# leijue222/Intra-and-Inter-Human-Relation-Network-for-MPEE

Measured on AMD Instinct MI355X. Metric: images/sec (256x192 crops) I2R-Net HRNet-W48 inference, higher is better.
Workload: dtype f32; 1 GPU; vanilla I2R-Net HRNet-W48-S 256x192, 6 encoder layers, fp32, random weights (BASELINE configs[1]: w48_pure_en6); images_per_gpu=8, persons_per_image=4, crops_per_gpu_step=32, parallelism=single GPU, programs_per_forward=3

## Files before the change

include/i2r_hip.h:

```cpp
#ifndef I2R_HIP_H
#define I2R_HIP_H

#include <stdint.h>

#ifdef __cplusplus
extern "C" {
#endif

#define I2R_ABI_VERSION 17

#define I2R_API __attribute__((visibility("default")))

#define I2R_OK 0
#define I2R_E_ARG (-1)
#define I2R_E_LAUNCH (-2)
#define I2R_E_NODEV (-3)

#define I2R_MAX_TAPS 9

typedef struct i2r_conv_desc {
    const float* in;
    const float* in2;
    const float* w;
    const float* bias;
    const float* res1;
    const float* res2;
    const float* res_post;
    float* out;
    int32_t n_img;
    int32_t in_h, in_w, in_cs;
    int32_t cin;
    int32_t conv_h, conv_w;
    int32_t out_h, out_w, out_cs;
    int32_t cout, cout_pad;
    int32_t stride;
    int32_t iy0, ix0;
    int32_t ntaps;
    int32_t dy[I2R_MAX_TAPS], dx[I2R_MAX_TAPS];
    int32_t out_step, out_off_y, out_off_x, rep;
    int32_t relu;
    int32_t tile_h, tile_w;
    int32_t ck;
    int32_t wn;
    int32_t mt;
    int32_t dtype;
    int32_t in_f16, out_f16;
    int32_t algo;
    int32_t t1_shift, t2_shift;
    const float* t1;
    const float* t2;
    float* y;
} i2r_conv_desc;

I2R_API int i2r_conv(const i2r_conv_desc* d, void* stream);

#define I2R_MAX_GROUP 4
I2R_API int i2r_conv_grouped(const i2r_conv_desc* const* descs, int32_t n, const int32_t* block_map, int32_t map_len,
                     void* stream);

I2R_API int i2r_stem_conv(const float* in_nchw, const float* w, const float* bias, float* out_nhwc, int32_t n_img,
                  int32_t cin, int32_t in_h, int32_t in_w, int32_t cout, int32_t out_cs, int32_t n_src, int32_t n_valid,
                  int32_t out_dt , void* stream);

I2R_API int i2r_pe_res_stem(const float* mask_nchw, const float* w_pre, const float* w7, const float* bias, float* out_nhwc,
                    int32_t n_img, int32_t in_h, int32_t in_w, int32_t cout, int32_t out_cs, int32_t n_src, int32_t n_valid, void* stream);

typedef struct i2r_pe_cat_vec_args {
    const float* in; const float* w; const float* bias; float* out;
    int32_t n_img, in_h, in_w, th, tw, rate, vec, out_cs, c0, c_end, n_src, n_valid;
} i2r_pe_cat_vec_args;
I2R_API int i2r_pe_cat_vec(const i2r_pe_cat_vec_args* a, void* stream);

I2R_API int i2r_maxpool3x3s2(const float* in, float* out, int32_t n_img, int32_t in_h, int32_t in_w, int32_t c,
                     int32_t in_cs, int32_t out_cs, void* stream);

I2R_API int i2r_head(const float* in, const float* w, const float* bias, float* out_nchw, int32_t n_img, int32_t h,
             int32_t w_, int32_t cin, int32_t in_cs, int32_t cout, void* stream);

I2R_API int i2r_conv_kernel_name(const i2r_conv_desc* const* descs, int32_t n, char* buf, int32_t buflen);

I2R_API int i2r_flip_merge(const float* y, const float* y_flipped, const int32_t* joint_map, float* out, int32_t n, int32_t joints,
                   int32_t h, int32_t w, void* stream);

I2R_API int i2r_decode(const float* heatmaps, const float* center, const float* scale, float* preds, float* maxvals, int32_t n,
               int32_t joints, int32_t h, int32_t w, int32_t blur_kernel, int32_t transform_back, void* stream);

typedef struct i2r_pose_nms_args {
    const float* preds; const float* maxvals; const float* scale; const float* area; const float* box_score;
    const int32_t* img_off; const float* sigmas;
    float* score; int32_t* rank; int32_t* n_keep;
    double in_vis_thre, oks_thre, oks_vis_thre;
    int32_t n_crops, n_img, joints, max_persons, soft, max_dets, use_oks_vis, reserved;
} i2r_pose_nms_args;
I2R_API int i2r_pose_nms(const i2r_pose_nms_args* a, void* stream);

I2R_API int i2r_group_nearest(const double* anchors, const int32_t* person_off, const int32_t* member_off, int32_t n_img, int32_t n_persons,
                              int32_t n_members, int32_t max_patch, int32_t* members, void* stream);

typedef struct i2r_oks_match_args {
    const float* dt_kpts; const float* dt_score; const uint8_t* dt_valid; const int32_t* dt_off;
    const double* gt_kpts; const double* gt_area; const double* gt_bbox; const int32_t* gt_flags; const int32_t* gt_off;
    const double* sigmas; const double* thr; const double* area_rng;
    int32_t* dt_rank; uint32_t* dt_match; uint32_t* dt_ignore; uint8_t* gt_ignore; double* oks; const int64_t* oks_off;
    int64_t oks_len;
    int32_t n_dt, n_gt, n_img, joints, n_thr, n_area, max_dets, max_dt_per_img, max_gt_per_img, reserved;
} i2r_oks_match_args;
I2R_API int i2r_oks_match(const i2r_oks_match_args* a, void* stream);

typedef struct i2r_oks_accumulate_args {
    const uint32_t* dt_match; const uint32_t* dt_ignore; const int32_t* dt_rank; const int32_t* order; const int32_t* dt_img;
    const int32_t* img_group; const uint8_t* gt_ignore; const int32_t* gt_off; const double* rec_thr;
    double* precision; double* recall; int32_t* npig;
    int32_t n_dt, n_gt, n_img, n_part, n_group, n_thr, n_area, n_rec;
} i2r_oks_accumulate_args;
I2R_API int i2r_oks_accumulate(const i2r_oks_accumulate_args* a, void* stream);

typedef struct i2r_joint_targets_args {
    const double* joints_hm; const float* joints_vis; const float* joints_weight;
    float* target_weight; float* target;
    double sigma;
    int32_t n_crops, joints, h, w;
} i2r_joint_targets_args;
I2R_API int i2r_joint_targets(const i2r_joint_targets_args* a, void* stream);

typedef struct i2r_val_metrics_args {
    const float* output;
    const float* target; const float* target_weight;
    const double* joints_hm; const float* joints_vis; const float* joints_weight;
    void* ws;
    double* loss; double* acc; double* avg_acc; int32_t* cnt; float* pred; double* sse; int32_t* hits; int32_t* valid; double* meter;
    double sigma;
    int32_t n_crops, joints, h, w, use_target_weight, reserved;
} i2r_val_metrics_args;
I2R_API int i2r_val_metrics(const i2r_val_metrics_args* a, void* stream);

I2R_API int i2r_crop_affine(const unsigned char* img, int32_t ih, int32_t iw, int32_t row_bytes, int32_t swap_rb, const float* inv_trans,
                    const float* mean, const float* inv_std, float* out, int32_t n, int32_t oh, int32_t ow, void* stream);

I2R_API int i2r_box_mask(const int32_t* boxes, int32_t ih, int32_t iw, float* out, int32_t n, int32_t oh, int32_t ow, void* stream);

I2R_API int i2r_crop_affine_cv2(const unsigned char* img, int32_t ih, int32_t iw, int32_t row_bytes, int32_t swap_rb, const double* inv_m,
                        const float* mean, const float* inv_std, float* out, int32_t n, int32_t oh, int32_t ow, void* stream);
I2R_API int i2r_box_mask_cv2(const int32_t* boxes, int32_t ih, int32_t iw, float* out, int32_t n, int32_t oh, int32_t ow, void* stream);

typedef struct {
    const unsigned char* img;
    int32_t ih, iw, row_bytes, reserved;
} i2r_image_ref;
typedef struct {
    double inv_m[6];
    int32_t box[4];
    int32_t image;
    int32_t reserved[3];
} i2r_crop_ref;
I2R_API int i2r_person_inputs_cv2(const i2r_image_ref* images, int32_t n_images, const i2r_crop_ref* crops, int32_t n_crops, int32_t swap_rb,
                          const float* mean, const float* inv_std, float* x_out, float* mask_out, int32_t oh, int32_t ow, void* stream);

I2R_API int i2r_layernorm(const float* in, const float* w, const float* b, float* out, int32_t npix, int32_t c, int32_t cs,
                  float eps, int32_t out_dt , void* stream);

I2R_API int i2r_window_attn(const float* qkv, const float* bias_qkv, float* out, int32_t n_img, int32_t h, int32_t w, int32_t c,
                    int32_t hs, int32_t heads, void* stream);

I2R_API int i2r_hrt_attn_block(const float* x, float* out, const float* ln_w, const float* ln_b, const void* wqkv, const float* bqkv,
                       const void* wo, const float* bo, int32_t n_img, int32_t h, int32_t w, int32_t c, int32_t cs, int32_t heads,
                       float eps, int32_t dtype, int32_t variant, void* stream);

I2R_API int i2r_hrt_mlp_block(const float* x, float* out, const float* ln_w, const float* ln_b, const void* w1, const float* b1,
                      const float* wdw, const float* bdw, const void* w2, const float* b2, int32_t n_img, int32_t h, int32_t w,
                      int32_t c, int32_t cs, int32_t hidden_pad, float eps, int32_t dtype, int32_t variant, void* stream);

I2R_API int i2r_dwconv3x3(const float* in, const float* w, const float* bias, float* out, int32_t n_img, int32_t in_h, int32_t in_w,
                  int32_t c, int32_t cs, int32_t stride, int32_t act, int32_t dt ,
                  void* stream);

I2R_API int i2r_upsample_bilinear_add(const float* low, const float* res, float* out, int32_t n_img, int32_t low_h, int32_t low_w,
                              int32_t scale, int32_t c, int32_t cs, int32_t act, void* stream);
struct i2r_up_args;
I2R_API int i2r_upsample_bilinear_add_multi(const struct i2r_up_args* a, void* stream);

I2R_API int i2r_fuse_up_add(const float* base, const float* t1, int32_t s1, const float* t2, int32_t s2, float* out, int32_t n_img,
                    int32_t h, int32_t w, int32_t cs, int32_t act, int32_t dt, void* stream);

typedef struct i2r_conv1x1_pair_args {
    const float* x; const float* w_a; const float* b_a; const float* res; float* y;
    const float* w_b; const float* b_b; float* z;
    int32_t n_pix, k_a, ca_out, cb_out, x_cs, y_cs, z_cs, relu_a, relu_b, mt;
} i2r_conv1x1_pair_args;
I2R_API int i2r_conv1x1_pair(const i2r_conv1x1_pair_args* a, void* stream);

typedef struct i2r_conv1x1_lp_args {
    const void* x; const void* w; const float* bias; const void* res1; const void* res_post; void* out;
    int32_t n_pix, cin_pad, cout_pad, x_cs, out_cs, act, dtype, in_16, out_16, mt;
    const void* res2;
} i2r_conv1x1_lp_args;
I2R_API int i2r_conv1x1_lp(const i2r_conv1x1_lp_args* a, void* stream);

typedef struct i2r_encoder_desc {
    const float* src;
    const float* pos;
    float* kbuf;
    float* vbuf;
    float* out;
    const int32_t* grp_off;
    const float* w_in;
    const float* b_in;
    const float* w_out;
    const float* b_out;
    const float* ln1_w; const float* ln1_b;
    const float* w1;
    const float* b1;
    const float* w2;
    const float* b2;
    const float* ln2_w; const float* ln2_b;
    int32_t n_tok, n_grp;
    int32_t d;
    int32_t cs;
    int32_t dff_pad;
    int32_t pos_period;
    int32_t n_qtiles32;
    float ln_eps;
    int32_t dtype;
    int32_t n_qtiles16, n_qtiles64;
    const void* w_in_lp; const void* w_out_lp; const void* w1_lp; const void* w2_lp;
    const float* next_w_in; const float* next_b_in; float* next_kbuf; float* next_vbuf;
    const float* vec_lp;
    float* split_ws; int32_t* split_cnt;
    int32_t n_qtiles192;
} i2r_encoder_desc;

I2R_API int i2r_encoder_kv(const i2r_encoder_desc* d, void* stream);
I2R_API int i2r_encoder_layer(const i2r_encoder_desc* d, void* stream);

typedef struct i2r_mh_attn_args {
    const float* qk; const float* v; float* out; const int32_t* grp_off;
    int32_t n_grp, heads, hp, k_off, qk_cs, v_cs, out_cs, n_qtiles16, n_qtiles32, n_qtiles64;
    const int32_t* key_len;
} i2r_mh_attn_args;
I2R_API int i2r_mh_attention(const i2r_mh_attn_args* a, void* stream);

typedef struct i2r_attn_weights_args {
    const float* qk; float* out; const int32_t* grp_off; const int64_t* out_off; float* ws;
    int32_t n_grp, heads, hp, k_off, qk_cs, n_tiles, ws_stride;
} i2r_attn_weights_args;
I2R_API int i2r_attn_weights(const i2r_attn_weights_args* a, void* stream);

typedef struct i2r_attn_query_args {
    const float* qk; float* out; const int32_t* grp_off; const int64_t* out_off; float* ws; const int32_t* q_tok; const int32_t* q_cnt;
    float* rows; const int32_t* grp_off_host;
    int32_t n_grp, heads, hp, k_off, qk_cs, n_tiles, ws_stride, mode, K, scale, h, w, n_col_tiles, reserved;
} i2r_attn_query_args;
I2R_API int i2r_attn_query_maps(const i2r_attn_query_args* a, void* stream);

I2R_API int i2r_rows_gather(const float* src, float* out, const int32_t* map, int32_t n_out, int32_t floats_per_crop, void* stream);
I2R_API int i2r_view_scramble(const float* o, float* out, const int32_t* person_map, int32_t n_out, int32_t n_images, int32_t max_persons, int32_t c,
                              int32_t cs, int32_t hw, void* stream);
typedef struct i2r_gather_args { const float* src; float* out; const int32_t* map; int32_t n_out, floats_per_crop; } i2r_gather_args;
typedef struct i2r_scramble_args { const float* o; float* out; const int32_t* person_map; int32_t n_out, n_images, max_persons, c, cs, hw; } i2r_scramble_args;

enum {
    I2R_OP_CONV = 1, I2R_OP_STEM = 2, I2R_OP_MAXPOOL = 3, I2R_OP_HEAD = 4,
    I2R_OP_ENC_KV = 5, I2R_OP_ENC_LAYER = 6, I2R_OP_FORK = 7, I2R_OP_JOIN = 8, I2R_OP_CONV_GROUP = 9,
    I2R_OP_LAYERNORM = 10, I2R_OP_WINATTN = 11, I2R_OP_DWCONV = 12, I2R_OP_UPSAMPLE = 13,
    I2R_OP_PE_RES_STEM = 15, I2R_OP_HRT_ATTN = 16, I2R_OP_HRT_MLP = 17,  I2R_OP_FUSE_UP = 19,
    I2R_OP_CONV1X1_PAIR = 20, I2R_OP_CONV1X1_LP = 21, I2R_OP_MH_ATTN = 22, I2R_OP_PE_CAT_VEC = 23, I2R_OP_ROWS_GATHER = 24, I2R_OP_VIEW_SCRAMBLE = 25,
    I2R_OP_RECORD = 26, I2R_OP_WAIT = 27, I2R_OP_LANE_FLAGS = 28, I2R_OP_ATTN_WEIGHTS = 29,
    I2R_OP_ATTN_QUERY = 30
};

typedef struct i2r_stem_args {
    const float* in; const float* w; const float* bias; float* out;
    int32_t n_img, cin, in_h, in_w, cout, out_cs, n_src, n_valid, out_dt;
} i2r_stem_args;

typedef struct i2r_pe_res_args {
    const float* in; const float* w_pre; const float* w7; const float* bias; float* out;
    int32_t n_img, in_h, in_w, cout, out_cs, n_src, n_valid;
} i2r_pe_res_args;

typedef struct i2r_pool_args {
    const float* in; float* out;
    int32_t n_img, in_h, in_w, c, in_cs, out_cs;
} i2r_pool_args;

typedef struct i2r_head_args {
    const float* in; const float* w; const float* bias; float* out;
    int32_t n_img, h, w_, cin, in_cs, cout;
} i2r_head_args;

typedef struct i2r_ln_args {
    const float* in; const float* w; const float* b; float* out;
    int32_t npix, c, cs; float eps; int32_t out_dt;
} i2r_ln_args;

typedef struct i2r_winattn_args {
    const float* qkv; const float* bias; float* out;
    int32_t n_img, h, w_, c, cs, heads;
} i2r_winattn_args;

typedef struct i2r_hrt_attn_args {
    const float* x; float* out; const float* ln_w; const float* ln_b; const void* wqkv; const float* bqkv; const void* wo; const float* bo;
    int32_t n_img, h, w_, c, cs, heads; float eps; int32_t dtype, variant;
} i2r_hrt_attn_args;

typedef struct i2r_hrt_mlp_args {
    const float* x; float* out; const float* ln_w; const float* ln_b; const void* w1; const float* b1; const float* wdw; const float* bdw;
    const void* w2; const float* b2;
    int32_t n_img, h, w_, c, cs, hidden_pad; float eps; int32_t dtype, variant;
} i2r_hrt_mlp_args;

typedef struct i2r_dw_args {
    const float* in; const float* w; const float* bias; float* out;
    int32_t n_img, in_h, in_w, c, cs, stride, act, dt;
} i2r_dw_args;

typedef struct i2r_up_args {
    const float* low; const float* res; float* out;
    int32_t n_img, low_h, low_w, scale, c, cs, act;
    const float* low2; const float* low3;
    int32_t scale2, scale3;
} i2r_up_args;

typedef struct i2r_fuse_up_args {
    const float* base; const float* t1; const float* t2; float* out;
    int32_t n_img, h, w, cs, s1, s2, act, dt;
} i2r_fuse_up_args;

typedef struct i2r_conv_group_args {
    const i2r_conv_desc* d[I2R_MAX_GROUP];
    const int32_t* block_map;
    int32_t n;
    int32_t map_len;
} i2r_conv_group_args;

typedef struct i2r_op {
    int32_t kind;
    int32_t lane;
    const void* args;
} i2r_op;

I2R_API int i2r_run_program(const i2r_op* ops, int32_t n_ops, void* const* streams, void* const* events);
I2R_API int i2r_run_program_timed(const i2r_op* ops, int32_t n_ops, void* const* streams, void* const* events, void* const* t0,
                                  void* const* t1);

I2R_API int i2r_abi_version(void);
I2R_API const char* i2r_last_error(void);
I2R_API int i2r_device_check(int32_t dev, int32_t* cu_count, int32_t* lds_bytes);

#ifdef __cplusplus
}
#endif
#endif
```

intra-and-inter-human-relation-network-for-mpee_amd/cabi.py:

```python
import ctypes as C
import os

import torch

_HERE = os.path.dirname(os.path.abspath(__file__))
LIB_PATH = os.path.join(_HERE, "libi2r_hip.so")

MAX_TAPS = 9
ABI_VERSION = 17
OP_CONV, OP_STEM, OP_MAXPOOL, OP_HEAD, OP_ENC_KV, OP_ENC_LAYER, OP_FORK, OP_JOIN, OP_CONV_GROUP = 1, 2, 3, 4, 5, 6, 7, 8, 9
MAX_GROUP = 4
OP_LAYERNORM, OP_WINATTN, OP_DWCONV, OP_UPSAMPLE = 10, 11, 12, 13
OP_CONV_CHAIN = 14
OP_PE_RES_STEM = 15
OP_HRT_ATTN = 16
OP_HRT_MLP = 17
OP_XSYNC = 18
OP_FUSE_UP = 19
OP_CONV1X1_PAIR = 20
OP_CONV1X1_LP = 21
OP_MH_ATTN = 22
OP_PE_CAT_VEC = 23
OP_ROWS_GATHER, OP_VIEW_SCRAMBLE = 24, 25
OP_RECORD, OP_WAIT = 26, 27
OP_LANE_FLAGS = 28
CAPTURE_OP_ATTN_WEIGHTS = 29
CAPTURE_OP_ATTN_QUERY = 30
SYNC_OPS = (OP_FORK, OP_JOIN, OP_XSYNC, OP_RECORD, OP_WAIT, OP_LANE_FLAGS)

_fp = C.c_void_p
_i32 = C.c_int32


class ConvDesc(C.Structure):
    _fields_ = [
        ("in_", _fp), ("in2", _fp), ("w", _fp), ("bias", _fp), ("res1", _fp), ("res2", _fp), ("res_post", _fp), ("out", _fp),
        ("n_img", _i32), ("in_h", _i32), ("in_w", _i32), ("in_cs", _i32), ("cin", _i32),
        ("conv_h", _i32), ("conv_w", _i32), ("out_h", _i32), ("out_w", _i32), ("out_cs", _i32),
        ("cout", _i32), ("cout_pad", _i32), ("stride", _i32), ("iy0", _i32), ("ix0", _i32), ("ntaps", _i32),
        ("dy", _i32 * MAX_TAPS), ("dx", _i32 * MAX_TAPS),
        ("out_step", _i32), ("out_off_y", _i32), ("out_off_x", _i32), ("rep", _i32), ("relu", _i32),
        ("tile_h", _i32), ("tile_w", _i32), ("ck", _i32), ("wn", _i32), ("mt", _i32), ("dtype", _i32),
        ("in_f16", _i32), ("out_f16", _i32), ("algo", _i32),
        ("t1_shift", _i32), ("t2_shift", _i32), ("t1", _fp), ("t2", _fp), ("y", _fp),
    ]


class EncoderDesc(C.Structure):
    _fields_ = [
        ("src", _fp), ("pos", _fp), ("kbuf", _fp), ("vbuf", _fp), ("out", _fp), ("grp_off", _fp),
        ("w_in", _fp), ("b_in", _fp), ("w_out", _fp), ("b_out", _fp), ("ln1_w", _fp), ("ln1_b", _fp),
        ("w1", _fp), ("b1", _fp), ("w2", _fp), ("b2", _fp), ("ln2_w", _fp), ("ln2_b", _fp),
        ("n_tok", _i32), ("n_grp", _i32), ("d", _i32), ("cs", _i32), ("dff_pad", _i32), ("pos_period", _i32),
        ("n_qtiles32", _i32), ("ln_eps", C.c_float), ("dtype", _i32), ("n_qtiles16", _i32), ("n_qtiles64", _i32),
        ("w_in_lp", _fp), ("w_out_lp", _fp), ("w1_lp", _fp), ("w2_lp", _fp),
        ("next_w_in", _fp), ("next_b_in", _fp), ("next_kbuf", _fp), ("next_vbuf", _fp), ("vec_lp", _fp),
        ("split_ws", _fp), ("split_cnt", _fp), ("n_qtiles192", _i32),
    ]


class StemArgs(C.Structure):
    _fields_ = [("in_", _fp), ("w", _fp), ("bias", _fp), ("out", _fp),
                ("n_img", _i32), ("cin", _i32), ("in_h", _i32), ("in_w", _i32), ("cout", _i32), ("out_cs", _i32), ("n_src", _i32),
                ("n_valid", _i32), ("out_dt", _i32)]


class PeResArgs(C.Structure):
    _fields_ = [("in_", _fp), ("w_pre", _fp), ("w7", _fp), ("bias", _fp), ("out", _fp),
                ("n_img", _i32), ("in_h", _i32), ("in_w", _i32), ("cout", _i32), ("out_cs", _i32), ("n_src", _i32), ("n_valid", _i32)]


class PeCatVecArgs(C.Structure):
    _fields_ = [("in_", _fp), ("w", _fp), ("bias", _fp), ("out", _fp),
                ("n_img", _i32), ("in_h", _i32), ("in_w", _i32), ("th", _i32), ("tw", _i32), ("rate", _i32), ("vec", _i32), ("out_cs", _i32),
                ("c0", _i32), ("c_end", _i32), ("n_src", _i32), ("n_valid", _i32)]


class PoolArgs(C.Structure):
    _fields_ = [("in_", _fp), ("out", _fp),
                ("n_img", _i32), ("in_h", _i32), ("in_w", _i32), ("c", _i32), ("in_cs", _i32), ("out_cs", _i32)]


class HeadArgs(C.Structure):
    _fields_ = [("in_", _fp), ("w", _fp), ("bias", _fp), ("out", _fp),
                ("n_img", _i32), ("h", _i32), ("w_", _i32), ("cin", _i32), ("in_cs", _i32), ("cout", _i32)]


class LnArgs(C.Structure):
    _fields_ = [("in_", _fp), ("w", _fp), ("b", _fp), ("out", _fp), ("npix", _i32), ("c", _i32), ("cs", _i32), ("eps", C.c_float),
                ("out_dt", _i32)]


class MhAttnArgs(C.Structure):
    _fields_ = [("qk", _fp), ("v", _fp), ("out", _fp), ("grp_off", _fp),
                ("n_grp", _i32), ("heads", _i32), ("hp", _i32), ("k_off", _i32), ("qk_cs", _i32), ("v_cs", _i32), ("out_cs", _i32),
                ("n_qtiles16", _i32), ("n_qtiles32", _i32), ("n_qtiles64", _i32), ("key_len", _fp)]


class AttnWeightsArgs(C.Structure):
    _fields_ = [("qk", _fp), ("out", _fp), ("grp_off", _fp), ("out_off", _fp), ("ws", _fp),
                ("n_grp", _i32), ("heads", _i32), ("hp", _i32), ("k_off", _i32), ("qk_cs", _i32), ("n_tiles", _i32), ("ws_stride", _i32)]


class AttnQueryArgs(C.Structure):
    _fields_ = [("qk", _fp), ("out", _fp), ("grp_off", _fp), ("out_off", _fp), ("ws", _fp), ("q_tok", _fp), ("q_cnt", _fp), ("rows", _fp),
                ("grp_off_host", _fp),
                ("n_grp", _i32), ("heads", _i32), ("hp", _i32), ("k_off", _i32), ("qk_cs", _i32), ("n_tiles", _i32), ("ws_stride", _i32),
                ("mode", _i32), ("K", _i32), ("scale", _i32), ("h", _i32), ("w", _i32), ("n_col_tiles", _i32), ("reserved", _i32)]


class GatherArgs(C.Structure):
    _fields_ = [("src", _fp), ("out", _fp), ("map", _fp), ("n_out", _i32), ("floats_per_crop", _i32)]


class ScrambleArgs(C.Structure):
    _fields_ = [("o", _fp), ("out", _fp), ("person_map", _fp), ("n_out", _i32), ("n_images", _i32), ("max_persons", _i32), ("c", _i32), ("cs", _i32),
                ("hw", _i32)]


class WinAttnArgs(C.Structure):
    _fields_ = [("qkv", _fp), ("bias", _fp), ("out", _fp),
                ("n_img", _i32), ("h", _i32), ("w_", _i32), ("c", _i32), ("cs", _i32), ("heads", _i32)]


class HrtAttnArgs(C.Structure):
    _fields_ = [("x", _fp), ("out", _fp), ("ln_w", _fp), ("ln_b", _fp), ("wqkv", _fp), ("bqkv", _fp), ("wo", _fp), ("bo", _fp),
                ("n_img", _i32), ("h", _i32), ("w_", _i32), ("c", _i32), ("cs", _i32), ("heads", _i32), ("eps", C.c_float), ("dtype", _i32),
                ("variant", _i32)]


class HrtMlpArgs(C.Structure):
    _fields_ = [("x", _fp), ("out", _fp), ("ln_w", _fp), ("ln_b", _fp), ("w1", _fp), ("b1", _fp), ("wdw", _fp), ("bdw", _fp), ("w2", _fp),
                ("b2", _fp), ("n_img", _i32), ("h", _i32), ("w_", _i32), ("c", _i32), ("cs", _i32), ("hidden_pad", _i32), ("eps", C.c_float),
                ("dtype", _i32), ("variant", _i32)]


class DwArgs(C.Structure):
    _fields_ = [("in_", _fp), ("w", _fp), ("bias", _fp), ("out", _fp),
                ("n_img", _i32), ("in_h", _i32), ("in_w", _i32), ("c", _i32), ("cs", _i32), ("stride", _i32), ("act", _i32), ("dt", _i32)]


class UpArgs(C.Structure):
    _fields_ = [("low", _fp), ("res", _fp), ("out", _fp),
                ("n_img", _i32), ("low_h", _i32), ("low_w", _i32), ("scale", _i32), ("c", _i32), ("cs", _i32), ("act", _i32),
                ("low2", _fp), ("low3", _fp), ("scale2", _i32), ("scale3", _i32)]


class FuseUpArgs(C.Structure):
    _fields_ = [("base", _fp), ("t1", _fp), ("t2", _fp), ("out", _fp),
                ("n_img", _i32), ("h", _i32), ("w", _i32), ("cs", _i32), ("s1", _i32), ("s2", _i32), ("act", _i32), ("dt", _i32)]


class Conv1x1PairArgs(C.Structure):
    _fields_ = [("x", _fp), ("w_a", _fp), ("b_a", _fp), ("res", _fp), ("y", _fp), ("w_b", _fp), ("b_b", _fp), ("z", _fp),
                ("n_pix", _i32), ("k_a", _i32), ("ca_out", _i32), ("cb_out", _i32), ("x_cs", _i32), ("y_cs", _i32), ("z_cs", _i32),
                ("relu_a", _i32), ("relu_b", _i32), ("mt", _i32)]


class Conv1x1LpArgs(C.Structure):
    _fields_ = [("x", _fp), ("w", _fp), ("bias", _fp), ("res1", _fp), ("res_post", _fp), ("out", _fp),
                ("n_pix", _i32), ("cin_pad", _i32), ("cout_pad", _i32), ("x_cs", _i32), ("out_cs", _i32), ("act", _i32), ("dtype", _i32),
                ("in_16", _i32), ("out_16", _i32), ("mt", _i32), ("res2", _fp)]


class ConvGroupArgs(C.Structure):
    _fields_ = [("d", C.POINTER(ConvDesc) * MAX_GROUP), ("block_map", _fp), ("n", _i32), ("map_len", _i32)]


class PoseNmsArgs(C.Structure):
    _fields_ = [("preds", _fp), ("maxvals", _fp), ("scale", _fp), ("area", _fp), ("box_score", _fp), ("img_off", _fp), ("sigmas", _fp),
                ("score", _fp), ("rank", _fp), ("n_keep", _fp),
                ("in_vis_thre", C.c_double), ("oks_thre", C.c_double), ("oks_vis_thre", C.c_double),
                ("n_crops", _i32), ("n_img", _i32), ("joints", _i32), ("max_persons", _i32), ("soft", _i32), ("max_dets", _i32),
                ("use_oks_vis", _i32), ("reserved", _i32)]


class OksMatchArgs(C.Structure):
    _fields_ = [("dt_kpts", _fp), ("dt_score", _fp), ("dt_valid", _fp), ("dt_off", _fp),
                ("gt_kpts", _fp), ("gt_area", _fp), ("gt_bbox", _fp), ("gt_flags", _fp), ("gt_off", _fp),
                ("sigmas", _fp), ("thr", _fp), ("area_rng", _fp),
                ("dt_rank", _fp), ("dt_match", _fp), ("dt_ignore", _fp), ("gt_ignore", _fp), ("oks", _fp), ("oks_off", _fp),
                ("oks_len", C.c_int64),
                ("n_dt", _i32), ("n_gt", _i32), ("n_img", _i32), ("joints", _i32), ("n_thr", _i32), ("n_area", _i32), ("max_dets", _i32),
                ("max_dt_per_img", _i32), ("max_gt_per_img", _i32), ("reserved", _i32)]


class OksAccumulateArgs(C.Structure):
    _fields_ = [("dt_match", _fp), ("dt_ignore", _fp), ("dt_rank", _fp), ("order", _fp), ("dt_img", _fp),
                ("img_group", _fp), ("gt_ignore", _fp), ("gt_off", _fp), ("rec_thr", _fp),
                ("precision", _fp), ("recall", _fp), ("npig", _fp),
                ("n_dt", _i32), ("n_gt", _i32), ("n_img", _i32), ("n_part", _i32), ("n_group", _i32), ("n_thr", _i32), ("n_area", _i32),
                ("n_rec", _i32)]


class JointTargetsArgs(C.Structure):
    _fields_ = [("joints_hm", _fp), ("joints_vis", _fp), ("joints_weight", _fp), ("target_weight", _fp), ("target", _fp),
                ("sigma", C.c_double), ("n_crops", _i32), ("joints", _i32), ("h", _i32), ("w", _i32)]


class ValMetricsArgs(C.Structure):
    _fields_ = [("output", _fp), ("target", _fp), ("target_weight", _fp), ("joints_hm", _fp), ("joints_vis", _fp), ("joints_weight", _fp),
                ("ws", _fp), ("loss", _fp), ("acc", _fp), ("avg_acc", _fp), ("cnt", _fp), ("pred", _fp), ("sse", _fp), ("hits", _fp),
                ("valid", _fp), ("meter", _fp), ("sigma", C.c_double),
                ("n_crops", _i32), ("joints", _i32), ("h", _i32), ("w", _i32), ("use_target_weight", _i32), ("reserved", _i32)]


class ImageRef(C.Structure):
    _fields_ = [("img", C.c_void_p), ("ih", _i32), ("iw", _i32), ("row_bytes", _i32), ("reserved", _i32)]


class CropRef(C.Structure):
    _fields_ = [("inv_m", C.c_double * 6), ("box", _i32 * 4), ("image", _i32), ("reserved", _i32 * 3)]


class Op(C.Structure):
    _fields_ = [("kind", _i32), ("lane", _i32), ("args", C.c_void_p)]


EXPORTS = ("i2r_conv", "i2r_conv_grouped", "i2r_conv_kernel_name", "i2r_stem_conv", "i2r_pe_res_stem", "i2r_maxpool3x3s2", "i2r_head", "i2r_layernorm", "i2r_window_attn", "i2r_hrt_attn_block", "i2r_hrt_mlp_block", "i2r_dwconv3x3",
           "i2r_upsample_bilinear_add", "i2r_upsample_bilinear_add_multi", "i2r_fuse_up_add", "i2r_conv1x1_pair", "i2r_conv1x1_lp", "i2r_flip_merge", "i2r_decode", "i2r_pose_nms", "i2r_group_nearest", "i2r_oks_match", "i2r_oks_accumulate", "i2r_joint_targets", "i2r_val_metrics", "i2r_crop_affine", "i2r_box_mask", "i2r_crop_affine_cv2", "i2r_box_mask_cv2", "i2r_person_inputs_cv2", "i2r_encoder_kv", "i2r_encoder_layer", "i2r_mh_attention", "i2r_attn_weights", "i2r_attn_query_maps", "i2r_pe_cat_vec", "i2r_rows_gather", "i2r_view_scramble",
           "i2r_run_program", "i2r_run_program_timed", "i2r_abi_version", "i2r_last_error", "i2r_device_check")

_LIB = None


class I2RError(RuntimeError):
    pass


def load_library(path=LIB_PATH):
    if not os.path.exists(path):
        raise I2RError(
            "HIP extension %s is missing -- build it with `python -c 'import __graft_entry__ as g; g.build()'`. "
            "There is no CPU fallback for the product path." % path)
    L = C.CDLL(path)
    L.i2r_conv.argtypes = [C.POINTER(ConvDesc), C.c_void_p]
    L.i2r_conv_grouped.argtypes = [C.POINTER(C.POINTER(ConvDesc)), _i32, _fp, _i32, C.c_void_p]
    L.i2r_conv_kernel_name.argtypes = [C.POINTER(C.POINTER(ConvDesc)), _i32, C.c_char_p, _i32]
    L.i2r_stem_conv.argtypes = [_fp, _fp, _fp, _fp, _i32, _i32, _i32, _i32, _i32, _i32, _i32, _i32, _i32, C.c_void_p]
    L.i2r_pe_res_stem.argtypes = [_fp, _fp, _fp, _fp, _fp, _i32, _i32, _i32, _i32, _i32, _i32, _i32, C.c_void_p]
    L.i2r_flip_merge.argtypes = [_fp, _fp, _fp, _fp, _i32, _i32, _i32, _i32, C.c_void_p]
    L.i2r_decode.argtypes = [_fp, _fp, _fp, _fp, _fp, _i32, _i32, _i32, _i32, _i32, _i32, C.c_void_p]
    L.i2r_pose_nms.argtypes = [C.POINTER(PoseNmsArgs), C.c_void_p]
    L.i2r_group_nearest.argtypes = [_fp, _fp, _fp, _i32, _i32, _i32, _i32, _fp, C.c_void_p]
    L.i2r_oks_match.argtypes = [C.POINTER(OksMatchArgs), C.c_void_p]
    L.i2r_oks_accumulate.argtypes = [C.POINTER(OksAccumulateArgs), C.c_void_p]
    L.i2r_joint_targets.argtypes = [C.POINTER(JointTargetsArgs), C.c_void_p]
    L.i2r_val_metrics.argtypes = [C.POINTER(ValMetricsArgs), C.c_void_p]
    L.i2r_crop_affine.argtypes = [_fp, _i32, _i32, _i32, _i32, _fp, _fp, _fp, _fp, _i32, _i32, _i32, C.c_void_p]
    L.i2r_box_mask.argtypes = [_fp, _i32, _i32, _fp, _i32, _i32, _i32, C.c_void_p]
    L.i2r_crop_affine_cv2.argtypes = [_fp, _i32, _i32, _i32, _i32, _fp, _fp, _fp, _fp, _i32, _i32, _i32, C.c_void_p]
    L.i2r_box_mask_cv2.argtypes = [_fp, _i32, _i32, _fp, _i32, _i32, _i32, C.c_void_p]
    L.i2r_person_inputs_cv2.argtypes = [_fp, _i32, _fp, _i32, _i32, C.POINTER(C.c_float), C.POINTER(C.c_float), _fp, _fp, _i32, _i32, C.c_void_p]
    L.i2r_fuse_up_add.argtypes = [_fp, _fp, _i32, _fp, _i32, _fp, _i32, _i32, _i32, _i32, _i32, _i32, C.c_void_p]
    L.i2r_conv1x1_pair.argtypes = [C.POINTER(Conv1x1PairArgs), C.c_void_p]
    L.i2r_conv1x1_lp.argtypes = [C.POINTER(Conv1x1LpArgs), C.c_void_p]
    L.i2r_maxpool3x3s2.argtypes = [_fp, _fp, _i32, _i32, _i32, _i32, _i32, _i32, C.c_void_p]
    L.i2r_head.argtypes = [_fp, _fp, _fp, _fp, _i32, _i32, _i32, _i32, _i32, _i32, C.c_void_p]
    L.i2r_layernorm.argtypes = [_fp, _fp, _fp, _fp, _i32, _i32, _i32, C.c_float, _i32, C.c_void_p]
    L.i2r_window_attn.argtypes = [_fp, _fp, _fp, _i32, _i32, _i32, _i32, _i32, _i32, C.c_void_p]
    L.i2r_hrt_attn_block.argtypes = [_fp, _fp, _fp, _fp, _fp, _fp, _fp, _fp, _i32, _i32, _i32, _i32, _i32, _i32, C.c_float, _i32, _i32, C.c_void_p]
    L.i2r_hrt_mlp_block.argtypes = [_fp] * 10 + [_i32] * 6 + [C.c_float, _i32, _i32, C.c_void_p]
    L.i2r_dwconv3x3.argtypes = [_fp, _fp, _fp, _fp, _i32, _i32, _i32, _i32, _i32, _i32, _i32, _i32, C.c_void_p]
    L.i2r_upsample_bilinear_add_multi.argtypes = [C.POINTER(UpArgs), C.c_void_p]
    L.i2r_upsample_bilinear_add.argtypes = [_fp, _fp, _fp, _i32, _i32, _i32, _i32, _i32, _i32, _i32, C.c_void_p]
    L.i2r_encoder_kv.argtypes = [C.POINTER(EncoderDesc), C.c_void_p]
    L.i2r_encoder_layer.argtypes = [C.POINTER(EncoderDesc), C.c_void_p]
    L.i2r_rows_gather.argtypes = [_fp, _fp, _fp, _i32, _i32, C.c_void_p]
    L.i2r_view_scramble.argtypes = [_fp, _fp, _fp, _i32, _i32, _i32, _i32, _i32, _i32, C.c_void_p]
    L.i2r_pe_cat_vec.argtypes = [C.POINTER(PeCatVecArgs), C.c_void_p]
    L.i2r_mh_attention.argtypes = [C.POINTER(MhAttnArgs), C.c_void_p]
    L.i2r_attn_weights.argtypes = [C.POINTER(AttnWeightsArgs), C.c_void_p]
    L.i2r_attn_query_maps.argtypes = [C.POINTER(AttnQueryArgs), C.c_void_p]
    L.i2r_run_program.argtypes = [C.POINTER(Op), _i32, C.POINTER(C.c_void_p), C.POINTER(C.c_void_p)]
    L.i2r_run_program_timed.argtypes = [C.POINTER(Op), _i32] + [C.POINTER(C.c_void_p)] * 4
    L.i2r_device_check.argtypes = [_i32, C.POINTER(_i32), C.POINTER(_i32)]
    L.i2r_last_error.restype = C.c_char_p
    for name in EXPORTS:
        if name != "i2r_last_error":
            getattr(L, name).restype = C.c_int
    return L


def lib():
    global _LIB
    if _LIB is None:
        L = load_library()
        if L.i2r_abi_version() != ABI_VERSION:
            raise I2RError("libi2r_hip.so ABI version %d != %d -- rebuild" % (L.i2r_abi_version(), ABI_VERSION))
        _LIB = L
    return _LIB


def check(rc, what=""):
    if rc != 0:
        msg = lib().i2r_last_error()
        raise I2RError("%s failed (rc=%d): %s" % (what or "i2r call", rc, msg.decode() if msg else "?"))


def require_gfx950(device_index=0):
    cu, lds = _i32(0), _i32(0)
    check(lib().i2r_device_check(device_index, C.byref(cu), C.byref(lds)), "i2r_device_check")
    return cu.value, lds.value
```

intra-and-inter-human-relation-network-for-mpee_amd/csrc/i2r_conv.h:

```cpp
#pragma once
#include "i2r_common.h"

#ifdef I2R_TUNING
#define I2R_DBG(p) ((p).dbg)
#else
#define I2R_DBG(p) 0
#endif

namespace {

struct ConvK {
    const float* in;
    const float* in2;
    const float* w;
    const float* bias;
    const float* res1;
    const float* res2;
    const float* res_post;
    float* out;
    int n_img, in_h, in_w, in_cs, cin;
    int conv_h, conv_w, out_h, out_w, out_cs, cout, cout_pad;
    int stride, iy0, ix0, ntaps;
    int tap_kh, tap_kw;
    int out_step, out_off_y, out_off_x, rep, relu;
    int tile_h, tile_w, tiles_y, tiles_x, n_cblk;
    int ph, pw, plane;
    int ck;
    int wn;
    int dtype;
    int in16, out16;
    int dbg;
    unsigned m_cblk, m_tx, m_ty, m_pw, m_tw;
    unsigned in_bytes, w_bytes, out_bytes;
    int wn_log, npass;
    int algo, w_fwlog, w_pitch, w_half, w_nfrag, w_rcp;
    int w_band;
    unsigned w_m_cblk, w_m_img, w_m_tx;
    const float* f_t1;
    const float* f_t2;
    float* f_y;
    int f_sh1, f_sh2;
    unsigned f_bytes1, f_bytes2;
};

__device__ __forceinline__ int div_m(int n, int d, unsigned m) { return d == 1 ? n : (int)__umulhi((unsigned)n, m); }

typedef unsigned u32x4 __attribute__((ext_vector_type(4)));
typedef unsigned u32x2 __attribute__((ext_vector_type(2)));
constexpr unsigned kOOB = 0x80000000u;
__device__ __forceinline__ __amdgpu_buffer_rsrc_t make_rsrc(const void* base, unsigned bytes) {
    return __builtin_amdgcn_make_buffer_rsrc(const_cast<void*>(base), 0, base ? bytes : 0, 0x00020000);
}
__device__ __forceinline__ f32x4 buf_ld16(const __amdgpu_buffer_rsrc_t& rs, unsigned voff, int soff) {
    return __builtin_bit_cast(f32x4, __builtin_amdgcn_raw_buffer_load_b128(rs, voff, soff, 0));
}
__device__ __forceinline__ void buf_st16(const __amdgpu_buffer_rsrc_t& rs, unsigned voff, int soff, f32x4 v) {
    __builtin_amdgcn_raw_buffer_store_b128(__builtin_bit_cast(u32x4, v), rs, voff, soff, 0);
    asm volatile("s_nop 1" ::"v"(v));
}

constexpr int kMaxPP = 5;

constexpr int kMaxGroups = 4;
struct ConvGroupK {
    ConvK g[kMaxGroups];
    int blk_end[kMaxGroups];
    int n;
    const int* blk_map;
};

template <int DT>
__device__ __forceinline__ f32x4 ld_act4(const float* base, size_t off, bool h16) {
    if constexpr (DT != 0) {
        if (h16) {
            const uint2 u = *reinterpret_cast<const uint2*>(reinterpret_cast<const unsigned short*>(base) + off);
            if constexpr (DT == 1)
                return (f32x4){__uint_as_float(u.x << 16), __uint_as_float(u.x & 0xFFFF0000u), __uint_as_float(u.y << 16), __uint_as_float(u.y & 0xFFFF0000u)};
            else {
                typedef _Float16 h4 __attribute__((ext_vector_type(4)));
                const h4 h = __builtin_bit_cast(h4, u);
                return (f32x4){(float)h[0], (float)h[1], (float)h[2], (float)h[3]};
            }
        }
    }
    return *reinterpret_cast<const f32x4*>(base + off);
}
template <int DT>
__device__ __forceinline__ void st_act4(float* base, size_t off, f32x4 v, bool h16) {
    if constexpr (DT != 0) {
        if (h16) {
            uint2 u;
            if constexpr (DT == 1) {
                typedef __bf16 b4 __attribute__((ext_vector_type(4)));
                const b4 b = {(__bf16)v[0], (__bf16)v[1], (__bf16)v[2], (__bf16)v[3]};
                u = __builtin_bit_cast(uint2, b);
            } else {
                typedef _Float16 h4 __attribute__((ext_vector_type(4)));
                const h4 h = {(_Float16)v[0], (_Float16)v[1], (_Float16)v[2], (_Float16)v[3]};
                u = __builtin_bit_cast(uint2, h);
            }
            *reinterpret_cast<uint2*>(reinterpret_cast<unsigned short*>(base) + off) = u;
            return;
        }
    }
    *reinterpret_cast<f32x4*>(base + off) = v;
}

template <int DT>
__device__ __forceinline__ f32x4 buf_ld_act4(const __amdgpu_buffer_rsrc_t& rs, unsigned voff, bool h16) {
    if constexpr (DT != 0) {
        if (h16) {
            const u32x2 u = __builtin_amdgcn_raw_buffer_load_b64(rs, voff, 0, 0);
            if constexpr (DT == 1)
                return (f32x4){__uint_as_float(u.x << 16), __uint_as_float(u.x & 0xFFFF0000u), __uint_as_float(u.y << 16), __uint_as_float(u.y & 0xFFFF0000u)};
            else {
                typedef _Float16 h4 __attribute__((ext_vector_type(4)));
                const h4 h = __builtin_bit_cast(h4, u);
                return (f32x4){(float)h[0], (float)h[1], (float)h[2], (float)h[3]};
            }
        }
    }
    return buf_ld16(rs, voff, 0);
}
template <int DT>
__device__ __forceinline__ void buf_st_act4(const __amdgpu_buffer_rsrc_t& rs, unsigned voff, f32x4 v, bool h16) {
    if constexpr (DT != 0) {
        if (h16) {
            u32x2 u;
            if constexpr (DT == 1) {
                typedef __bf16 b4 __attribute__((ext_vector_type(4)));
                const b4 b = {(__bf16)v[0], (__bf16)v[1], (__bf16)v[2], (__bf16)v[3]};
                u = __builtin_bit_cast(u32x2, b);
            } else {
                typedef _Float16 h4 __attribute__((ext_vector_type(4)));
                const h4 h = {(_Float16)v[0], (_Float16)v[1], (_Float16)v[2], (_Float16)v[3]};
                u = __builtin_bit_cast(u32x2, h);
            }
            __builtin_amdgcn_raw_buffer_store_b64(u, rs, voff, 0, 0);
            return;
        }
    }
    __builtin_amdgcn_raw_buffer_store_b128(__builtin_bit_cast(u32x4, v), rs, voff, 0, 0);
}

template <int MT, int NT, int DT>
__device__ __forceinline__ void conv_epilogue(const ConvK& p, f32x4 (&acc)[MT][NT], int img, int oy0, int ox0, int wm, int n_base,
                                              int li, int g, int tile_px) {
    if ((I2R_DBG(p) & 1) && acc[0][0][0] != 12345.678f) return;
    const int j4 = li & 3;
    const int pj = li >> 2, pq = li & 3;
    const int perm_src = (g * 16 + pq * 4 + pj) * 4;
    auto to_pixel_major = [&](f32x4 v) {
        v = quad_transpose(v, j4);
#pragma unroll
        for (int e = 0; e < 4; ++e) {
            const float x = v[e];
            v[e] = __int_as_float(__builtin_amdgcn_ds_bpermute(perm_src, __float_as_int(x)));
        }
        return v;
    };
    const bool h16 = DT != 0 && p.out16;
    const unsigned esz = h16 ? 2u : 4u;
    const __amdgpu_buffer_rsrc_t rs_out = make_rsrc(p.out, p.out_bytes), rs_r1 = make_rsrc(p.res1, p.out_bytes),
                                 rs_r2 = make_rsrc(p.res2, p.out_bytes), rs_rp = make_rsrc(p.res_post, p.out_bytes);
    auto finish = [&](f32x4 t, int n, bool full, unsigned voff) {
        if (p.relu == 1) {
            t[0] = fmaxf(t[0], 0.f); t[1] = fmaxf(t[1], 0.f); t[2] = fmaxf(t[2], 0.f); t[3] = fmaxf(t[3], 0.f);
        } else if (p.relu == 2) {
#pragma unroll
            for (int e = 0; e < 4; ++e) t[e] = 0.5f * t[e] * (1.f + erff(t[e] * 0.70710678118654752f));
        }
        if (p.res_post) t += buf_ld_act4<DT>(rs_rp, voff, h16);
        if (!full) {
#pragma unroll
            for (int e = 0; e < 4; ++e)
                if (n + e >= p.cout) t[e] = 0.f;
        }
        return t;
    };
    f32x4 bias[NT];
    unsigned noff[NT];
    const bool tail = n_base + NT * 16 > p.cout || n_base + NT * 16 > p.out_cs;
#pragma unroll
    for (int nt = 0; nt < NT; ++nt) {
        const int n = n_base + nt * 16 + pq * 4;
        const bool nok = n < p.cout_pad && (n + 4 <= p.cout || n + 4 <= p.out_cs);
        noff[nt] = nok ? (unsigned)n * esz : kOOB;
        bias[nt] = n < p.cout_pad ? *reinterpret_cast<const f32x4*>(p.bias + n) : (f32x4){0.f, 0.f, 0.f, 0.f};
    }
    if (p.rep == 1 && !(I2R_DBG(p) & 16)) {
        unsigned off[MT];
#pragma unroll
        for (int mt = 0; mt < MT; ++mt) {
            const int m = (wm * MT + mt) * 16 + g * 4 + pj;
            const int ty = div_m(m, p.tile_w, p.m_tw), tx = m - ty * p.tile_w;
            const int oy = oy0 + ty, ox = ox0 + tx;
            const bool pv = m < tile_px && oy < p.conv_h && ox < p.conv_w;
            off[mt] = pv ? (unsigned)(((img * p.out_h + oy * p.out_step + p.out_off_y) * p.out_w + ox * p.out_step + p.out_off_x) * p.out_cs) * esz : kOOB;
        }
        auto at = [&](int mt, int nt) { return (tail && noff[nt] == kOOB) ? kOOB : off[mt] + noff[nt]; };
        f32x4 r[MT][NT];
#pragma unroll
        for (int mt = 0; mt < MT; ++mt)
#pragma unroll
            for (int nt = 0; nt < NT; ++nt) {
                r[mt][nt] = bias[nt];
                if (p.res1) r[mt][nt] += buf_ld_act4<DT>(rs_r1, at(mt, nt), h16);
                if (p.res2) r[mt][nt] += buf_ld_act4<DT>(rs_r2, at(mt, nt), h16);
            }
#pragma unroll
        for (int mt = 0; mt < MT; ++mt)
#pragma unroll
            for (int nt = 0; nt < NT; ++nt) {
                const f32x4 v = to_pixel_major(acc[mt][nt]);
                const int n = n_base + nt * 16 + pq * 4;
                const unsigned o = at(mt, nt);
                buf_st_act4<DT>(rs_out, o, finish(v + r[mt][nt], n, !tail || n + 4 <= p.cout, o), h16);
            }
        return;
    }
#pragma unroll
    for (int mt = 0; mt < MT; ++mt) {
        const int m = (wm * MT + mt) * 16 + g * 4 + pj;
        const int ty = div_m(m, p.tile_w, p.m_tw), tx = m - ty * p.tile_w;
        const int oy = oy0 + ty, ox = ox0 + tx;
        const bool pvalid = m < tile_px && oy < p.conv_h && ox < p.conv_w;
        const int by = oy * p.out_step + p.out_off_y, bx = ox * p.out_step + p.out_off_x;
#pragma unroll
        for (int nt = 0; nt < NT; ++nt) {
            const f32x4 v = to_pixel_major(acc[mt][nt]) + bias[nt];
            const int n = n_base + nt * 16 + pq * 4;
            if (!pvalid || noff[nt] == kOOB) continue;
            for (int ry = 0; ry < p.rep; ++ry)
                for (int rx = 0; rx < p.rep; ++rx) {
                    const unsigned o = (unsigned)(((img * p.out_h + by + ry) * p.out_w + bx + rx) * p.out_cs) * esz + noff[nt];
                    f32x4 t = v;
                    if (p.res1) t += buf_ld_act4<DT>(rs_r1, o, h16);
                    if (p.res2) t += buf_ld_act4<DT>(rs_r2, o, h16);
                    buf_st_act4<DT>(rs_out, o, finish(t, n, n + 4 <= p.cout, o), h16);
                }
        }
    }
}



typedef void (*conv_fn)(const ConvGroupK);

}

void* i2r_pick_conv_bf16(int nt, int mt, int cap, int pf);
void* i2r_pick_conv_f16(int nt, int mt, int cap, int pf);
void* i2r_pick_conv_wino(int nt, int mt, int fin);
size_t i2r_conv_wino_lds(int nt, int mt, int plane);
```

intra-and-inter-human-relation-network-for-mpee_amd/csrc/i2r_conv.hip:

```cpp
#include <stdlib.h>

#include <algorithm>

#include "i2r_conv.h"

namespace {

template <int MT, int NT, int CAP, int PF>
__device__ __forceinline__ void conv_body(const ConvK& p, int bid, f32x4* lds) {
    const int tid = threadIdx.x;
    unsigned long long ts0 = 0, ts1 = 0, ts2 = 0;
    const bool stamp = (I2R_DBG(p) & 8) != 0;
    const int bid_stamp = bid;
    if (stamp) ts0 = __builtin_amdgcn_s_memtime();
    const int lane = tid & 63, wave = tid >> 6;
    const int WN = p.wn;
    const int wm = wave >> p.wn_log, wn = wave & (WN - 1);
    const int li = lane & 15, g = lane >> 4;

    int q = div_m(bid, p.n_cblk, p.m_cblk);
    const int cb = bid - q * p.n_cblk;
    bid = q;
    q = div_m(bid, p.tiles_x, p.m_tx);
    const int tile_x = bid - q * p.tiles_x;
    bid = q;
    const int img = div_m(bid, p.tiles_y, p.m_ty);
    const int tile_y = bid - img * p.tiles_y;
    const int oy0 = tile_y * p.tile_h, ox0 = tile_x * p.tile_w;
    const int py0 = oy0 * p.stride + p.iy0, px0 = ox0 * p.stride + p.ix0;
    const int phw = p.ph * p.pw;

    constexpr int NPP = PF > 0 ? 4 * PF : kMaxPP;
    const int ul = tid & 3;
    const __amdgpu_buffer_rsrc_t rs_in = make_rsrc(p.in, p.in_bytes), rs_in2 = make_rsrc(p.in2, p.in_bytes), rs_w = make_rsrc(p.w, p.w_bytes);
    unsigned goff[NPP];
#pragma unroll
    for (int j = 0; j < NPP; ++j) {
        const int pp = PF > 0 ? (tid >> 2) + j * 64 : tid + j * 256;
        goff[j] = kOOB;
        if (pp < phw) {
            const int py = div_m(pp, p.pw, p.m_pw), px = pp - py * p.pw;
            const int iy = py0 + py, ix = px0 + px;
            if (iy >= 0 && iy < p.in_h && ix >= 0 && ix < p.in_w) goff[j] = (unsigned)(((img * p.in_h + iy) * p.in_w + ix) * p.in_cs) * 4u;
        }
    }
    const int npp = (phw + 255) >> 8;

    const int tile_px = p.tile_h * p.tile_w;
    int ppix[MT];
#pragma unroll
    for (int mt = 0; mt < MT; ++mt) {
        int m = (wm * MT + mt) * 16 + li;
        if (m >= tile_px) m = 0;
        const int ty = div_m(m, p.tile_w, p.m_tw), tx = m - ty * p.tile_w;
        ppix[mt] = ty * p.stride * p.pw + tx * p.stride;
    }

    f32x4 acc[MT][NT];
#pragma unroll
    for (int mt = 0; mt < MT; ++mt)
#pragma unroll
        for (int nt = 0; nt < NT; ++nt) acc[mt][nt] = (f32x4){0.f, 0.f, 0.f, 0.f};

    const int n_base = (cb * WN + wn) * NT * 16;
    const int cin4 = p.cin >> 2;
    const unsigned wlane = (unsigned)(n_base + li + g * p.cout_pad) * 16u;

    auto run_chunk = [&](const f32x4* buf, int c0, int ckc, auto&& mid) {
        const int ncs = ckc >> 4;
        const int nit = p.ntaps * ncs;
        const int wp0 = (c0 >> 2) * p.cout_pad * 16;
        int wp = wp0;
        const int inc_cs = 4 * p.cout_pad * 16;
        const int inc_tap = (cin4 - (ncs - 1) * 4) * p.cout_pad * 16;
        int cs_n = 0, tx_n = 0, ty_n = 0;
        auto fetch = [&](f32x4(&a)[MT], f32x4(&b)[NT]) {
#pragma unroll
            for (int nt = 0; nt < NT; ++nt) b[nt] = buf_ld16(rs_w, wlane + nt * 256u, (I2R_DBG(p) & 4) ? wp0 : wp);
            const int abase = (cs_n * 4 + g) * p.plane + ty_n * p.pw + tx_n;
#pragma unroll
            for (int mt = 0; mt < MT; ++mt) a[mt] = buf[abase + ppix[mt]];
            if (++cs_n == ncs) {
                cs_n = 0;
                wp += inc_tap;
                if (++tx_n == p.tap_kw) {
                    tx_n = 0;
                    if (++ty_n == p.tap_kh) { ty_n = 0; wp = wp0; }
                }
            } else {
                wp += inc_cs;
            }
        };
        auto fma_step = [&](const f32x4(&a)[MT], const f32x4(&b)[NT]) {
#pragma unroll
            for (int s = 0; s < 4; ++s)
#pragma unroll
                for (int mt = 0; mt < MT; ++mt)
#pragma unroll
                    for (int nt = 0; nt < NT; ++nt) acc[mt][nt] = mfma16(a[mt][s], b[nt][s], acc[mt][nt]);
        };
        f32x4 a0[MT], a1[MT], b0[NT], b1[NT];
        fetch(a0, b0);
        mid();
        int it = 0;
        for (; it + 2 <= nit; it += 2) {
            fetch(a1, b1);
            fma_step(a0, b0);
            fetch(a0, b0);
            fma_step(a1, b1);
        }
        if (it < nit) fma_step(a0, b0);
    };

    if constexpr (PF > 0) {
        constexpr int UQ = CAP / 4, PJ = 4 * PF;
        f32x4 v[UQ][PJ];
        const int ckg = p.ck >> 2;
        auto stage_load = [&](int c0) {
#pragma unroll
            for (int uq = 0; uq < UQ; ++uq)
                if (uq * 4 < ckg) {
#pragma unroll
                    for (int j = 0; j < PJ; ++j)
                        v[uq][j] = (I2R_DBG(p) & 2) ? (f32x4){0.f, 0.f, 0.f, 0.f} : buf_ld16(rs_in, goff[j] + (uq * 4 + ul) * 16u, c0 * 4);
                }
            if (p.in2) {
#pragma unroll
                for (int uq = 0; uq < UQ; ++uq)
                    if (uq * 4 < ckg) {
#pragma unroll
                        for (int j = 0; j < PJ; ++j)
                            v[uq][j] += buf_ld16(rs_in2, goff[j] + (uq * 4 + ul) * 16u, c0 * 4);
                    }
            }
        };
        auto stage_store = [&](f32x4* buf) {
#pragma unroll
            for (int uq = 0; uq < UQ; ++uq)
                if (uq * 4 < ckg) {
#pragma unroll
                    for (int j = 0; j < PJ; ++j) {
                        const int pp = (tid >> 2) + j * 64;
                        if (pp < phw) buf[(uq * 4 + ul) * p.plane + pp] = v[uq][j];
                    }
                }
        };
        const int npass = p.npass;
        stage_load(0);
        stage_store(lds);
        __syncthreads();
        if (stamp) ts1 = __builtin_amdgcn_s_memtime();
        for (int pass = 0; pass < npass; ++pass) {
            f32x4* cur = lds + (pass & 1) * ckg * p.plane;
            f32x4* nxt = lds + ((pass + 1) & 1) * ckg * p.plane;
            const bool more = pass + 1 < npass;
            run_chunk(cur, pass * p.ck, p.ck, [&]() { if (more) stage_load((pass + 1) * p.ck); });
            if (more) stage_store(nxt);
            __syncthreads();
        }
    } else {
        for (int c0 = 0; c0 < p.cin; c0 += p.ck) {
            const int ckc = min(p.ck, p.cin - c0);
            const int ncg = ckc >> 2;
            if (c0 != 0) __syncthreads();
            for (int cg0 = 0; cg0 < ncg; cg0 += 4) {
                f32x4 v[4][kMaxPP];
#pragma unroll
                for (int u = 0; u < 4; ++u)
#pragma unroll
                    for (int j = 0; j < kMaxPP; ++j)
                        v[u][j] = (j < npp && !(I2R_DBG(p) & 2)) ? buf_ld16(rs_in, goff[j] + u * 16u, (c0 + cg0 * 4) * 4) : (f32x4){0.f, 0.f, 0.f, 0.f};
                if (p.in2) {
#pragma unroll
                    for (int u = 0; u < 4; ++u)
#pragma unroll
                        for (int j = 0; j < kMaxPP; ++j)
                            if (j < npp) v[u][j] += buf_ld16(rs_in2, goff[j] + u * 16u, (c0 + cg0 * 4) * 4);
                }
#pragma unroll
                for (int u = 0; u < 4; ++u)
#pragma unroll
                    for (int j = 0; j < kMaxPP; ++j) {
                        const int pp = tid + j * 256;
                        if (j < npp && pp < phw)
                            lds[(cg0 + u) * p.plane + pp] = v[u][j];
                    }
            }
            __syncthreads();
            run_chunk(lds, c0, ckc, []() {});
        }
    }

    if (stamp) {
        ts2 = __builtin_amdgcn_s_memtime();
        ConvK q = p;
        q.res2 = nullptr;
        conv_epilogue<MT, NT, 0>(q, acc, img, oy0, ox0, wm, n_base, li, g, tile_px);
        asm volatile("s_waitcnt vmcnt(0)" ::: "memory");
        const unsigned long long ts3 = __builtin_amdgcn_s_memtime();
        if (tid == 0) {
            unsigned long long* o = reinterpret_cast<unsigned long long*>(const_cast<float*>(p.res2)) + (size_t)bid_stamp * 4;
            o[0] = ts0; o[1] = ts1; o[2] = ts2; o[3] = ts3;
            if (I2R_DBG(p) & 32) {
                const unsigned hw = __builtin_amdgcn_s_getreg((4 << 0) | (0 << 6) | (31 << 11));
                const unsigned xcc = __builtin_amdgcn_s_getreg((20 << 0) | (0 << 6) | (3 << 11));
                o[1] = ((unsigned long long)xcc << 32) | hw;
            }
        }
        return;
    }
    conv_epilogue<MT, NT, 0>(p, acc, img, oy0, ox0, wm, n_base, li, g, tile_px);
}

template <int MT, int NT, int CAP, int PF>
__global__ __launch_bounds__(256) void conv_igemm_f32(const ConvGroupK grp) {
    extern __shared__ __attribute__((aligned(16))) f32x4 lds[];
    int bid = blockIdx.x, gi = 0, start = 0;
    if (grp.blk_map) {
        const int v = __builtin_amdgcn_readfirstlane(grp.blk_map[bid]);
        gi = v >> 24;
        bid = v & 0xFFFFFF;
    } else {
#pragma unroll
        for (int i = 0; i < kMaxGroups - 1; ++i)
            if (i + 1 < grp.n && bid >= grp.blk_end[i]) { gi = i + 1; start = grp.blk_end[i]; }
    }
    conv_body<MT, NT, CAP, PF>(grp.g[gi], bid - start, lds);
}

template <int NT, int CAP, int PF>
conv_fn pick_mt(int mt) {
    switch (mt) {
        case 1: return conv_igemm_f32<1, NT, CAP, PF>;
        case 2: return conv_igemm_f32<2, NT, CAP, PF>;
        case 3: return conv_igemm_f32<3, NT, CAP, PF>;
        case 4: return conv_igemm_f32<4, NT, CAP, PF>;
    }
    return nullptr;
}

template <int CAP, int PF>
conv_fn pick_nt(int nt, int mt) {
    switch (nt) {
        case 3: return pick_mt<3, CAP, PF>(mt);
        case 4: return pick_mt<4, CAP, PF>(mt);
        case 5: return pick_mt<5, CAP, PF>(mt);
    }
    return nullptr;
}

conv_fn pick_kernel(int nt, int mt, int cap, int pf) {
    if (pf == 0) return pick_nt<4, 0>(nt, mt);
    if (pf == 1 && cap == 4) return pick_nt<4, 1>(nt, mt);
    if (pf == 1 && cap == 12) return pick_nt<12, 1>(nt, mt);
    if (pf == 2 && cap == 4) return pick_nt<4, 2>(nt, mt);
    return nullptr;
}

inline int cdiv(int a, int b) { return (a + b - 1) / b; }

}

static void copy_desc(const i2r_conv_desc* d, ConvK& k) {
    k.in = d->in; k.in2 = d->in2; k.w = d->w; k.bias = d->bias; k.res1 = d->res1; k.res2 = d->res2; k.res_post = d->res_post; k.out = d->out;
    k.n_img = d->n_img; k.in_h = d->in_h; k.in_w = d->in_w; k.in_cs = d->in_cs; k.cin = d->cin;
    k.conv_h = d->conv_h; k.conv_w = d->conv_w; k.out_h = d->out_h; k.out_w = d->out_w; k.out_cs = d->out_cs;
    k.cout = d->cout; k.cout_pad = d->cout_pad; k.stride = d->stride; k.iy0 = d->iy0; k.ix0 = d->ix0;
    k.ntaps = d->ntaps;
    k.out_step = d->out_step; k.out_off_y = d->out_off_y; k.out_off_x = d->out_off_x; k.rep = d->rep; k.relu = d->relu;
    k.dtype = d->dtype;
    k.in16 = d->in_f16; k.out16 = d->out_f16;
    k.algo = d->algo; k.w_fwlog = k.w_pitch = k.w_half = k.w_nfrag = k.w_rcp = k.w_band = 0;
    k.w_m_cblk = k.w_m_img = k.w_m_tx = 0; k.in_bytes = k.w_bytes = k.out_bytes = 0;
    k.m_cblk = k.m_tx = k.m_ty = k.m_pw = k.m_tw = 0; k.wn_log = 0; k.npass = 0;
    k.dbg = 0;
    k.f_t1 = d->t1; k.f_t2 = d->t2; k.f_y = d->y; k.f_sh1 = d->t1_shift; k.f_sh2 = d->t2 ? d->t2_shift : 0; k.f_bytes1 = k.f_bytes2 = 0;
}

static int prepare_wino(const i2r_conv_desc* d, int force_mt, ConvK& k, int* nt_out, int* mt_out, int* cap_out, int* pf_out, size_t* lds_out,
                        long long* nblk_out) {
    I2R_CHECK_ARG(d->dtype == 0 && !d->in_f16 && !d->out_f16, "i2r_conv: the Winograd kernels are fp32");
    I2R_CHECK_ARG(d->stride == 1 && d->ntaps == 9 && d->iy0 == -1 && d->ix0 == -1 && d->rep == 1 && d->out_step == 1 && d->out_off_y == 0 &&
                      d->out_off_x == 0 && d->in2 == nullptr,
                  "i2r_conv: algo 1 (Winograd) needs a plain 3x3 stride-1 pad-1 convolution");
    for (int t = 0; t < 9; ++t) I2R_CHECK_ARG(d->dy[t] == t / 3 && d->dx[t] == t % 3, "i2r_conv: algo 1 needs row-major 3x3 taps");
    I2R_CHECK_ARG(d->relu == 0 || d->relu == 1, "i2r_conv: algo 1 has no GELU epilogue");
    I2R_CHECK_ARG((long long)d->n_img * d->in_h * d->in_w * d->in_cs < (1ll << 29) && (long long)d->n_img * d->out_h * d->out_w * d->out_cs < (1ll << 29) &&
                      (long long)16 * d->cin * d->cout_pad < (1ll << 29),
                  "i2r_conv: algo 1 addresses its tensors through buffer descriptors of < 2 GiB");
    I2R_CHECK_ARG(d->conv_h == d->in_h && d->conv_w == d->in_w && d->out_h == d->conv_h && d->out_w == d->conv_w, "i2r_conv: algo 1 geometry");
    if (d->t1) {
        I2R_CHECK_ARG(d->y != nullptr, "i2r_conv: a fused input (t1) needs y");
        I2R_CHECK_ARG(d->in_cs == d->cin, "i2r_conv: fused input: y is complete only when the conv reads every channel (cin=%d in_cs=%d)", d->cin, d->in_cs);
        for (int t = 0; t < (d->t2 ? 2 : 1); ++t) {
            const int sh = t ? d->t2_shift : d->t1_shift;
            I2R_CHECK_ARG((sh == 1 || sh == 2) && d->in_h % (1 << sh) == 0 && d->in_w % (1 << sh) == 0,
                          "i2r_conv: fused input: t%d_shift %d must be 1 or 2 and the %dx%d map divisible by the scale", t + 1, sh, d->in_h, d->in_w);
        }
        const void* others[] = {d->in, d->t1, d->t2, d->out, d->res1, d->res2, d->res_post};
        for (const void* o : others) I2R_CHECK_ARG((const void*)d->y != o, "i2r_conv: fused input: y aliases another tensor of the launch");
        I2R_CHECK_ARG(d->t1 != (const float*)d->out && d->t2 != (const float*)d->out, "i2r_conv: out aliases a fused-input term");
    }
    const int nfrag = d->cout_pad / 16;
    const int nt = nfrag % 3 == 0 ? 3 : (nfrag % 4 == 0 ? 4 : 0);
    I2R_CHECK_ARG(nt != 0, "i2r_conv: algo 1 needs cout_pad=%d to be a multiple of 48 or 64", d->cout_pad);
    const int mt = force_mt ? force_mt : (d->mt ? d->mt : 1);
    I2R_CHECK_ARG(mt == 1, "i2r_conv: algo 1 takes mt 1 (got %d)", mt);
    int fw = 0;
    if (d->tile_w) {
        I2R_CHECK_ARG(d->tile_w == 16 || d->tile_w == 8 || d->tile_w == 4, "i2r_conv: algo 1 fragment width %d (16, 8, 4)", d->tile_w);
        fw = d->tile_w / 2;
    } else {
        long long best = -1;
        for (int cand : {8, 4, 2}) {
            const long long n = (long long)cdiv(d->conv_w, 2 * cand) * cdiv(d->conv_h, 32 / cand);
            if (best < 0 || n < best) { best = n; fw = cand; }
        }
    }
    copy_desc(d, k);
    k.w_fwlog = fw == 8 ? 3 : (fw == 4 ? 2 : 1);
    k.tile_w = 2 * fw; k.tile_h = 32 / fw;
    k.tiles_x = cdiv(d->conv_w, k.tile_w); k.tiles_y = cdiv(d->conv_h, k.tile_h);
    k.n_cblk = nfrag / nt;
    k.ph = k.tile_h + 2; k.pw = k.tile_w + 2;
    k.w_half = fw + 1;
    k.w_pitch = fw == 8 ? 20 : (fw == 4 ? 10 : 9);
    k.plane = cdiv(k.ph * k.w_pitch, 16) * 16;
    k.w_rcp = (65536 + k.pw - 1) / k.pw;
    k.in_bytes = (unsigned)((long long)d->n_img * d->in_h * d->in_w * d->in_cs * 4);
    k.w_bytes = (unsigned)((long long)16 * d->cin * d->cout_pad * 4);
    k.out_bytes = (unsigned)((long long)d->n_img * d->out_h * d->out_w * d->out_cs * 4);
    if (d->t1) k.f_bytes1 = (unsigned)((long long)d->n_img * (d->in_h >> d->t1_shift) * (d->in_w >> d->t1_shift) * d->in_cs * 4);
    if (d->t2) k.f_bytes2 = (unsigned)((long long)d->n_img * (d->in_h >> d->t2_shift) * (d->in_w >> d->t2_shift) * d->in_cs * 4);
    auto magic = [](int d) { return d == 1 ? 0u : (unsigned)(((1ull << 32) + d - 1) / d); };
    k.w_m_cblk = magic(k.n_cblk); k.w_m_img = magic(k.tiles_y * k.tiles_x); k.w_m_tx = magic(k.tiles_x);
    k.tap_kw = k.tap_kh = 3;
    k.ck = 16; k.wn = 1;
    const long long nf = (long long)d->n_img * k.tiles_y * k.tiles_x;
    I2R_CHECK_ARG(nf > 0 && nf * k.n_cblk < (1ll << 20) && k.tiles_y * k.tiles_x < 2048 && k.n_cblk < 2048, "i2r_conv: algo 1 grid (%lld fragments)", nf);
    k.w_nfrag = (int)nf;
#ifdef I2R_TUNING
    {
        static const int dbg = getenv("I2R_CONV_DBG") ? atoi(getenv("I2R_CONV_DBG")) : 0;
        k.dbg = dbg;
    }
#endif
    *nt_out = nt; *mt_out = mt; *cap_out = 0; *pf_out = 100;
    *lds_out = i2r_conv_wino_lds(nt, mt, k.plane);
    *nblk_out = (nf + mt - 1) / mt * k.n_cblk;
    return I2R_OK;
}

static int prepare(const i2r_conv_desc* d, int force_mt, int force_cap, int force_pf, ConvK& k, int* nt_out, int* mt_out, int* cap_out,
                   int* pf_out, size_t* lds_out, long long* nblk_out) {
    I2R_CHECK_ARG(d && d->in && d->w && d->bias && d->out, "i2r_conv: null pointer");
    I2R_CHECK_ARG(d->cin > 0 && d->cin % 16 == 0 && d->cin <= d->in_cs && d->in_cs % 4 == 0,
                  "i2r_conv: cin=%d must be a multiple of 16 and <= in_cs=%d (in_cs %% 4 == 0)", d->cin, d->in_cs);
    I2R_CHECK_ARG(d->cout > 0 && d->cout_pad % 16 == 0 && d->cout <= d->cout_pad && d->cout <= d->out_cs && d->out_cs % 4 == 0,
                  "i2r_conv: cout=%d cout_pad=%d out_cs=%d", d->cout, d->cout_pad, d->out_cs);
    I2R_CHECK_ARG(d->stride == 1 || d->stride == 2, "i2r_conv: stride %d", d->stride);
    I2R_CHECK_ARG(d->dtype >= 0 && d->dtype <= 2 && (d->dtype == 0 || d->in2 == nullptr), "i2r_conv: dtype %d", d->dtype);
    I2R_CHECK_ARG((d->in_f16 == 0 || d->in_f16 == 1) && (d->out_f16 == 0 || d->out_f16 == 1) && (d->dtype != 0 || (!d->in_f16 && !d->out_f16)),
                  "i2r_conv: 16-bit activation storage (in_f16=%d out_f16=%d) needs a 16-bit operand type (dtype=%d)", d->in_f16, d->out_f16, d->dtype);
    I2R_CHECK_ARG(!d->in_f16 || d->in_cs % 8 == 0, "i2r_conv: 16-bit input needs in_cs %% 8 == 0 (in_cs=%d)", d->in_cs);
    I2R_CHECK_ARG(d->ntaps >= 1 && d->ntaps <= I2R_MAX_TAPS, "i2r_conv: ntaps %d", d->ntaps);
    I2R_CHECK_ARG(d->rep >= 1 && d->out_step >= 1, "i2r_conv: rep/out_step");
    I2R_CHECK_ARG((d->conv_h - 1) * d->out_step + d->out_off_y + d->rep <= d->out_h &&
                      (d->conv_w - 1) * d->out_step + d->out_off_x + d->rep <= d->out_w,
                  "i2r_conv: destination grid exceeds out tensor");
    I2R_CHECK_ARG(d->in2 != (const float*)d->out && d->in != (const float*)d->out, "i2r_conv: out aliases in");
    I2R_CHECK_ARG(d->algo == 0 || d->algo == 1, "i2r_conv: algo %d", d->algo);
    I2R_CHECK_ARG(d->t1 ? d->algo == 1 : (!d->t2 && !d->y), "i2r_conv: a fused input (t1, t2, y) needs algo 1 and starts with t1");
    if (d->algo == 1) return prepare_wino(d, force_mt, k, nt_out, mt_out, cap_out, pf_out, lds_out, nblk_out);

    int max_dy = 0, max_dx = 0;
    for (int t = 0; t < d->ntaps; ++t) {
        I2R_CHECK_ARG(d->dy[t] >= 0 && d->dx[t] >= 0, "i2r_conv: negative tap offset");
        if (d->dy[t] > max_dy) max_dy = d->dy[t];
        if (d->dx[t] > max_dx) max_dx = d->dx[t];
    }

    const int nfrag = d->cout_pad / 16;
    int nt = 0;
    for (int cand : {3, 4, 5})
        if (nfrag % cand == 0) { nt = cand; break; }
    I2R_CHECK_ARG(nt != 0, "i2r_conv: cout_pad=%d is not a multiple of 48, 64 or 80", d->cout_pad);
    int wn = d->wn;
    if (wn == 0) {
        const int nb = nfrag / nt;
        wn = (nb % 4 == 0) ? 4 : (nb % 2 == 0) ? 2 : 1;
        if (wn == 4 && d->cout_pad < 192) wn = 2;
    }
    I2R_CHECK_ARG((wn == 1 || wn == 2 || wn == 4) && (nfrag / nt) % wn == 0, "i2r_conv: wn=%d does not divide cout", wn);
    const int wm = 4 / wn;

    int th = d->tile_h, tw = d->tile_w, mt = force_mt ? force_mt : d->mt;
    if (th == 0 || tw == 0) {
        tw = d->conv_w <= 16 ? d->conv_w : (d->conv_w % 16 == 0 ? 16 : (d->conv_w % 12 == 0 ? 12 : 8));
        if (mt == 0) mt = 2;
        th = (wm * mt * 16) / tw;
        if (th < 1) th = 1;
        if (th > d->conv_h) th = d->conv_h;
    }
    if (mt == 0) mt = cdiv(th * tw, wm * 16);
    I2R_CHECK_ARG(mt >= 1 && mt <= 4 && th * tw <= wm * mt * 16, "i2r_conv: tile %dx%d does not fit wm=%d mt=%d", th, tw, wm, mt);

    copy_desc(d, k);
    k.tile_h = th; k.tile_w = tw;
    k.tiles_y = cdiv(d->conv_h, th); k.tiles_x = cdiv(d->conv_w, tw);
    k.n_cblk = nfrag / (nt * wn);
    k.ph = (th - 1) * d->stride + max_dy + 1;
    k.pw = (tw - 1) * d->stride + max_dx + 1;
    I2R_CHECK_ARG(k.ph * k.pw <= kMaxPP * 256, "i2r_conv: patch %dx%d too large", k.ph, k.pw);
#ifdef I2R_TUNING
    static const int plane_pad = getenv("I2R_CONV_PLANE_PAD") ? atoi(getenv("I2R_CONV_PLANE_PAD")) : 0;
#else
    constexpr int plane_pad = 0;
#endif
    k.plane = cdiv(k.ph * k.pw, 16) * 16 + plane_pad;
    k.tap_kw = max_dx + 1;
    k.tap_kh = max_dy + 1;
    for (int t = 0; t < d->ntaps; ++t)
        I2R_CHECK_ARG(d->dy[t] == t / k.tap_kw && d->dx[t] == t % k.tap_kw && d->ntaps == (max_dy + 1) * (max_dx + 1),
                      "i2r_conv: taps must form a dense row-major kh x kw grid");
    const int npp = cdiv(k.ph * k.pw, 256);
#ifdef I2R_TUNING
    static const int pf_env = getenv("I2R_CONV_PF") ? atoi(getenv("I2R_CONV_PF")) : 1;
#else
    constexpr int pf_env = 1;
#endif
    const int cin_g = d->dtype == 0 ? d->cin / 4 : (d->cin / 8 + 3) / 4 * 4;
    const int g_ch = d->dtype == 0 ? 4 : 8;
    int pf = (pf_env && d->ck == 0 && npp <= 2 && cin_g % 4 == 0) ? npp : 0;
    int cap = 4;
    if (force_pf >= 0) {
        I2R_CHECK_ARG(force_pf == 0 || (npp <= force_pf && d->ck == 0 && cin_g % 4 == 0), "i2r_conv: grouped members disagree on the staging mode");
        pf = force_pf;
    }
    int ck = d->ck;
    size_t lds_bytes;
    if (pf > 0) {
        int ckg = 4;
#ifdef I2R_TUNING
        static const int cap_env = getenv("I2R_CONV_CAP") ? atoi(getenv("I2R_CONV_CAP")) : 12;
#else
        constexpr int cap_env = 12;
#endif
        const int cap_max = std::min(cap_env, d->dtype == 0 ? 12 : 8);
        const int cap_lim = force_pf >= 0 ? force_cap : (pf == 1 ? cap_max : 4);
        for (int cand : {12, 8, 4})
            if (cand <= cap_lim && cin_g % cand == 0 && (size_t)2 * cand * k.plane * 16 <= 40 * 1024) { ckg = cand; break; }
        cap = force_pf >= 0 ? force_cap : (ckg > 4 ? cap_max : 4);
        ck = ckg * g_ch;
        lds_bytes = (size_t)2 * ckg * k.plane * 16;
    } else if (d->dtype != 0) {
        const int g8_pad = (d->cin / 8 + 3) / 4 * 4;
        int fit = (24 * 1024 / (k.plane * 16)) / 4 * 4;
        if (fit < 4) fit = 4;
        const int nchunk = cdiv(g8_pad, fit);
        const int ckg = cdiv(cdiv(g8_pad, nchunk), 4) * 4;
        ck = ckg * 8;
        lds_bytes = (size_t)ckg * k.plane * 16;
    } else {
        if (ck == 0) {
            const int budget = 20 * 1024;
            int fit = (budget / (k.plane * 16)) * 4;
            fit = fit < 16 ? 16 : fit / 16 * 16;
            const int nchunk = cdiv(d->cin, fit);
            ck = cdiv(cdiv(d->cin, nchunk), 16) * 16;
        }
        I2R_CHECK_ARG(ck % 16 == 0 && ck >= 16, "i2r_conv: ck=%d", ck);
        lds_bytes = (size_t)(ck / 4) * k.plane * 16;
    }
    k.ck = ck;
    I2R_CHECK_ARG(lds_bytes <= 160 * 1024, "i2r_conv: LDS %zu B", lds_bytes);
    k.wn = wn;
    {
        const long long esz_in = d->in_f16 ? 2 : 4, esz_out = d->out_f16 ? 2 : 4;
        const long long inb = (long long)d->n_img * d->in_h * d->in_w * d->in_cs * esz_in, outb = (long long)d->n_img * d->out_h * d->out_w * d->out_cs * esz_out;
        const long long wb = d->dtype == 0 ? (long long)d->ntaps * d->cin * d->cout_pad * 4 : (long long)d->ntaps * ((d->cin / 8 + 3) / 4 * 4) * 8 * d->cout_pad * 2;
        I2R_CHECK_ARG(inb < (1ll << 31) && outb < (1ll << 31) && wb < (1ll << 31), "i2r_conv: tensors of 2 GiB and more are not supported (in %lld, out %lld, weights %lld bytes)", inb, outb, wb);
        k.in_bytes = (unsigned)inb; k.out_bytes = (unsigned)outb; k.w_bytes = (unsigned)wb;
        auto magic = [](int d) { return d == 1 ? 0u : (unsigned)(((1ull << 32) + d - 1) / d); };
        k.m_cblk = magic(k.n_cblk); k.m_tx = magic(k.tiles_x); k.m_ty = magic(k.tiles_y); k.m_pw = magic(k.pw); k.m_tw = magic(k.tile_w);
        k.wn_log = wn == 4 ? 2 : (wn == 2 ? 1 : 0);
        k.npass = d->dtype == 0 ? d->cin / ck : ((d->cin / 8 + 3) / 4 * 4) / (ck / 8);
    }
#ifdef I2R_TUNING
    {
        static const int dbg = getenv("I2R_CONV_DBG") ? atoi(getenv("I2R_CONV_DBG")) : 0;
        k.dbg = dbg;
    }
#endif
    const long long nblk = (long long)d->n_img * k.tiles_y * k.tiles_x * k.n_cblk;
    I2R_CHECK_ARG(nblk > 0 && nblk < (1ll << 30), "i2r_conv: grid");
    I2R_CHECK_ARG(nblk * std::max(k.n_cblk, std::max(k.tiles_x, k.tiles_y)) < (1ll << 32) && (long long)kMaxPP * 256 * k.pw < (1ll << 32),
                  "i2r_conv: grid of %lld workgroups exceeds the index-decode range", nblk);
    *nt_out = nt; *mt_out = mt; *cap_out = cap; *pf_out = pf; *lds_out = lds_bytes; *nblk_out = nblk;
    return I2R_OK;
}

static int resolve(const i2r_conv_desc* const* descs, int32_t n, ConvGroupK& grp, int* nt0_, int* mt0_, int* cap0_, int* pf0_,
                   size_t* lds_, long long* total_, bool table = true) {
    I2R_CHECK_ARG(descs && n >= 1 && n <= kMaxGroups, "i2r_conv_grouped: 1..%d descriptors", kMaxGroups);
    int nt0 = 0, mt0 = 0, pf0 = -1, cap0 = 4;
    size_t lds_max = 0;
    long long total = 0;
    for (int i = 0; i < n; ++i) I2R_CHECK_ARG(descs[i] && descs[i]->algo == descs[0]->algo, "i2r_conv_grouped: members mix algorithms");
    if (n > 1 && descs[0]->algo == 0) {
        pf0 = 0;
        cap0 = 4;
        bool all_pf = true;
        for (int i = 0; i < n; ++i) {
            ConvK tmp;
            int nt, mt, cap, pf;
            size_t lds;
            long long nblk;
            int rc = prepare(descs[i], mt0, 4, -1, tmp, &nt, &mt, &cap, &pf, &lds, &nblk);
            if (rc) return rc;
            if (i == 0) mt0 = mt;
            if (pf == 0) all_pf = false;
            if (pf > pf0) pf0 = pf;
            if (cap > cap0) cap0 = cap;
        }
        if (!all_pf) pf0 = 0;
        if (pf0 != 1) cap0 = 4;
        mt0 = 0;
    }
    for (int i = 0; i < n; ++i) {
        int nt, mt, cap, pf;
        size_t lds;
        long long nblk;
        int rc = prepare(descs[i], mt0, cap0, pf0, grp.g[i], &nt, &mt, &cap, &pf, &lds, &nblk);
        if (rc) return rc;
        if (i == 0) { nt0 = nt; mt0 = mt; pf0 = pf; cap0 = cap; }
        I2R_CHECK_ARG(nt == nt0 && mt == mt0, "i2r_conv_grouped: descriptor %d has fragment blocking (%d,%d) != (%d,%d)", i, mt, nt, mt0, nt0);
        I2R_CHECK_ARG(descs[i]->dtype == descs[0]->dtype, "i2r_conv_grouped: members mix compute dtypes");
        if (lds > lds_max) lds_max = lds;
        if (descs[i]->algo == 1 && !table) {
            const long long groups = nblk / grp.g[i].n_cblk;
            grp.g[i].w_band = (int)((groups + 7) / 8);
            nblk = (long long)grp.g[i].w_band * 8 * grp.g[i].n_cblk;
        }
        total += nblk;
        grp.blk_end[i] = (int)total;
    }
    for (int i = n; i < kMaxGroups; ++i) { grp.g[i] = grp.g[0]; grp.blk_end[i] = (int)total; }
    grp.n = n;
    I2R_CHECK_ARG(total < (1ll << 31), "i2r_conv_grouped: grid");
    *nt0_ = nt0; *mt0_ = mt0; *cap0_ = cap0; *pf0_ = pf0; *lds_ = lds_max; *total_ = total;
    return I2R_OK;
}

static bool any_fused_input(const i2r_conv_desc* const* descs, int32_t n) {
    for (int i = 0; i < n; ++i)
        if (descs[i]->t1) return true;
    return false;
}

extern "C" int i2r_conv_grouped(const i2r_conv_desc* const* descs, int32_t n, const int32_t* block_map,
                                int32_t map_len, void* stream) {
    ConvGroupK grp;
    int nt0, mt0, cap0, pf0;
    size_t lds_max;
    long long total;
    int rc = resolve(descs, n, grp, &nt0, &mt0, &cap0, &pf0, &lds_max, &total, block_map != nullptr);
    if (rc) return rc;
    grp.blk_map = block_map;
    I2R_CHECK_ARG(block_map == nullptr || map_len == (int32_t)total, "i2r_conv_grouped: block_map has %d entries, grid has %lld", map_len, total);
    conv_fn fn = descs[0]->algo == 1 ? reinterpret_cast<conv_fn>(i2r_pick_conv_wino(nt0, mt0, any_fused_input(descs, n)))
                 : descs[0]->dtype == 0 ? pick_kernel(nt0, mt0, cap0, pf0)
                                      : reinterpret_cast<conv_fn>(descs[0]->dtype == 1 ? i2r_pick_conv_bf16(nt0, mt0, cap0, pf0) : i2r_pick_conv_f16(nt0, mt0, cap0, pf0));
    I2R_CHECK_ARG(fn != nullptr, "i2r_conv: no kernel for nt=%d mt=%d cap=%d pf=%d dtype=%d", nt0, mt0, cap0, pf0, descs[0]->dtype);
    if (lds_max > 64 * 1024)
        (void)hipFuncSetAttribute(reinterpret_cast<const void*>(fn), hipFuncAttributeMaxDynamicSharedMemorySize, (int)lds_max);
    const unsigned grid = (unsigned)total;
    i2r_launch(fn, dim3(grid), dim3(256), lds_max, (hipStream_t)stream, grp);
    I2R_CHECK_LAUNCH("i2r_conv");
    return I2R_OK;
}

extern "C" int i2r_conv(const i2r_conv_desc* d, void* stream) { return i2r_conv_grouped(&d, 1, nullptr, 0, stream); }

extern "C" int i2r_conv_kernel_name(const i2r_conv_desc* const* descs, int32_t n, char* buf, int32_t buflen) {
    ConvGroupK grp;
    int nt0, mt0, cap0, pf0;
    size_t lds_max;
    long long total;
    int rc = resolve(descs, n, grp, &nt0, &mt0, &cap0, &pf0, &lds_max, &total);
    if (rc) return rc;
    I2R_CHECK_ARG(buf && buflen > 0, "i2r_conv_kernel_name: buffer");
    if (descs[0]->algo == 1)
        snprintf(buf, (size_t)buflen, "conv_wino_%sf32<%d, %d>", any_fused_input(descs, n) ? "fin_" : "", mt0, nt0);
    else if (descs[0]->dtype)
        snprintf(buf, (size_t)buflen, "conv_igemm_lp<%d, %d, %d, %d>/%s", mt0, nt0, cap0, pf0, descs[0]->dtype == 1 ? "bf16" : "f16");
    else
        snprintf(buf, (size_t)buflen, "conv_igemm_f32<%d, %d, %d, %d>", mt0, nt0, cap0, pf0);
    return I2R_OK;
}
```

intra-and-inter-human-relation-network-for-mpee_amd/csrc/i2r_conv_wino.hip:

```cpp
#include "i2r_conv.h"

namespace {

constexpr int kWinoPatchMax = 108;

template <int MT, int NT, bool FIN>
__device__ __forceinline__ void conv_wino_body(const ConvGroupK& grp) {
    extern __shared__ __attribute__((aligned(16))) f32x4 lds[];
    const int tid = threadIdx.x, lane = tid & 63;
    const int wi = __builtin_amdgcn_readfirstlane(tid >> 6);
    const int li = lane & 15, g = lane >> 4;

    int bid = blockIdx.x, gi = 0;
    if (grp.blk_map) {
        const int v = __builtin_amdgcn_readfirstlane(grp.blk_map[bid]);
        gi = v >> 24;
        bid = v & 0xFFFFFF;
    } else {
        int start = 0;
#pragma unroll
        for (int i = 0; i < kMaxGroups - 1; ++i)
            if (i + 1 < grp.n && bid >= grp.blk_end[i]) { gi = i + 1; start = grp.blk_end[i]; }
        bid -= start;
    }
    const ConvK& p = grp.g[gi];
    const bool stamp = (I2R_DBG(p) & 8) != 0;
    unsigned long long ts0 = 0, ts1 = 0, ts2 = 0;
    if (stamp) ts0 = __builtin_amdgcn_s_memtime();
    const float* const res2 = stamp ? nullptr : p.res2;

    int wg, cb;
    if (grp.blk_map) {
        wg = div_m(bid, p.n_cblk, p.w_m_cblk);
        cb = bid - wg * p.n_cblk;
    } else {
        const int q = bid >> 3, qq = div_m(q, p.n_cblk, p.w_m_cblk);
        cb = q - qq * p.n_cblk;
        wg = (bid & 7) * p.w_band + qq;
        if (wg * MT >= p.w_nfrag) return;
    }
    const int fwl = p.w_fwlog, FW = 1 << fwl;
    const int PC = p.pw, PP = p.ph * p.pw;
    const int per_img = p.tiles_y * p.tiles_x;
    const int pitch = p.w_pitch, half = p.w_half, plane = p.plane;
    const int n_base = cb * NT * 16;
    int f_img[MT], f_oy[MT], f_ox[MT];
    bool f_ok[MT];
#pragma unroll
    for (int mt = 0; mt < MT; ++mt) {
        int fid = wg * MT + mt;
        f_ok[mt] = fid < p.w_nfrag;
        if (!f_ok[mt]) fid = 0;
        f_img[mt] = div_m(fid, per_img, p.w_m_img);
        const int rem = fid - f_img[mt] * per_img;
        const int fy = div_m(rem, p.tiles_x, p.w_m_tx);
        f_oy[mt] = fy * (32 >> fwl);
        f_ox[mt] = (rem - fy * p.tiles_x) * (2 * FW);
    }

    constexpr int NIT = (MT * kWinoPatchMax * 4 + 255) / 256;
    const __amdgpu_buffer_rsrc_t rs_in = __builtin_amdgcn_make_buffer_rsrc(const_cast<float*>(p.in), 0, p.in_bytes, 0x00020000);
    const __amdgpu_buffer_rsrc_t rs_w = __builtin_amdgcn_make_buffer_rsrc(const_cast<float*>(p.w), 0, p.w_bytes, 0x00020000);
    unsigned goff[NIT];
    int lslot[NIT];
    const bool fin = FIN && p.f_t1 != nullptr, fin2 = fin && p.f_t2 != nullptr;
    const __amdgpu_buffer_rsrc_t rs_t1 = make_rsrc(fin ? p.f_t1 : nullptr, p.f_bytes1), rs_t2 = make_rsrc(fin2 ? p.f_t2 : nullptr, p.f_bytes2),
                                 rs_y = make_rsrc(fin ? p.f_y : nullptr, p.in_bytes);
    unsigned goff1[FIN ? NIT : 1], goff2[FIN ? NIT : 1];
    bool own[FIN ? NIT : 1];
#pragma unroll
    for (int k = 0; k < NIT; ++k) {
        const int it = tid + k * 256;
        const int cg = it & 3, pix = it >> 2;
        int f = 0, pp = pix;
#pragma unroll
        for (int m = 1; m <= MT; ++m)
            if (pix >= m * PP) { f = m; pp = pix - m * PP; }
        const int row = (pp * p.w_rcp) >> 16, col = pp - row * PC;
        goff[k] = kOOB;
        lslot[k] = -1;
        if constexpr (FIN) { goff1[k] = goff2[k] = kOOB; own[k] = false; }
        if (f < MT) {
            int img = f_img[0], oy = f_oy[0], ox = f_ox[0];
            bool ok = f_ok[0];
#pragma unroll
            for (int m = 1; m < MT; ++m)
                if (f == m) { img = f_img[m]; oy = f_oy[m]; ox = f_ox[m]; ok = f_ok[m]; }
            const int iy = oy - 1 + row, ix = ox - 1 + col;
            lslot[k] = (f * 4 + cg) * plane + row * pitch + (col & 1) * half + (col >> 1);
            if (ok && iy >= 0 && iy < p.in_h && ix >= 0 && ix < p.in_w) {
                goff[k] = (unsigned)(((img * p.in_h + iy) * p.in_w + ix) * p.in_cs + cg * 4) * 4u;
                if constexpr (FIN) {
                    const int s1 = p.f_sh1, s2 = p.f_sh2;
                    goff1[k] = (unsigned)(((img * (p.in_h >> s1) + (iy >> s1)) * (p.in_w >> s1) + (ix >> s1)) * p.in_cs + cg * 4) * 4u;
                    goff2[k] = (unsigned)(((img * (p.in_h >> s2) + (iy >> s2)) * (p.in_w >> s2) + (ix >> s2)) * p.in_cs + cg * 4) * 4u;
                    own[k] = row >= 1 && row < p.ph - 1 && col >= 1 && col < PC - 1;
                }
            }
        }
    }
    f32x4 v[NIT];
    auto stage_load = [&](int c0) {
#pragma unroll
        for (int k = 0; k < NIT; ++k)
            v[k] = (I2R_DBG(p) & 2) ? (f32x4){0.f, 0.f, 0.f, 0.f}
                                    : __builtin_bit_cast(f32x4, __builtin_amdgcn_raw_buffer_load_b128(rs_in, goff[k], c0 * 4, 0));
    };
    f32x4 vt[FIN ? NIT : 1];
    auto stage_load_t1 = [&](int c0) {
        if constexpr (FIN) {
            if (fin) {
#pragma unroll
                for (int k = 0; k < NIT; ++k) vt[k] = buf_ld16(rs_t1, goff1[k], c0 * 4);
            }
        }
    };
    auto stage_mid = [&](int c0) {
        if constexpr (FIN) {
            if (fin2) {
#pragma unroll
                for (int k = 0; k < NIT; ++k) {
                    v[k] += vt[k];
                    vt[k] = buf_ld16(rs_t2, goff2[k], c0 * 4);
                }
            }
        }
    };
    auto stage_store = [&](f32x4* buf, int c0) {
        if constexpr (FIN) {
            if (fin) {
#pragma unroll
                for (int k = 0; k < NIT; ++k) {
                    v[k] += vt[k];
                    v[k][0] = fmaxf(v[k][0], 0.f); v[k][1] = fmaxf(v[k][1], 0.f); v[k][2] = fmaxf(v[k][2], 0.f); v[k][3] = fmaxf(v[k][3], 0.f);
                    if (cb == 0) buf_st16(rs_y, own[k] ? goff[k] : kOOB, c0 * 4, v[k]);
                }
            }
        }
#pragma unroll
        for (int k = 0; k < NIT; ++k)
            if (lslot[k] >= 0) buf[lslot[k]] = v[k];
    };

    const int ra = wi == 0 ? 0 : (wi == 2 ? 2 : 1);
    const int rb = wi == 0 ? 2 : (wi == 1 ? 2 : (wi == 2 ? 1 : 3));
    const float sg = wi == 1 ? 1.f : -1.f;
    const int ty = li >> fwl, tx = li & (FW - 1);
    const int abase = g * plane + 2 * ty * pitch + tx;
    const int oa = ra * pitch, ob = rb * pitch;
    auto load_a = [&](const f32x4* buf, f32x4 (&a)[MT][4]) {
#pragma unroll
        for (int mt = 0; mt < MT; ++mt) {
            const f32x4* q = buf + mt * 4 * plane + abase;
            f32x4 R[4];
#pragma unroll
            for (int c = 0; c < 4; ++c) {
                const int oc = (c & 1) * half + (c >> 1);
                const f32x4 xa = q[oa + oc], xb = q[ob + oc];
                R[c] = xa + sg * xb;
            }
            a[mt][0] = R[0] - R[2];
            a[mt][1] = R[1] + R[2];
            a[mt][2] = R[2] - R[1];
            a[mt][3] = R[1] - R[3];
        }
    };

    const int cin4 = p.cin >> 2;
    const unsigned wlane = (unsigned)(n_base + li + g * p.cout_pad) * 16u;
    int wp = wi * 4 * cin4 * p.cout_pad * 16;
    const int inc_j = cin4 * p.cout_pad * 16;
    const int inc_wrap = (4 - 3 * cin4) * p.cout_pad * 16;
    auto fetch_b = [&](f32x4 (&b)[NT]) {
#pragma unroll
        for (int nt = 0; nt < NT; ++nt)
            b[nt] = __builtin_bit_cast(f32x4, __builtin_amdgcn_raw_buffer_load_b128(rs_w, wlane + nt * 256u, (I2R_DBG(p) & 4) ? 0 : wp, 0));
    };

    f32x4 acc[4][MT][NT];
    const int npass = p.cin >> 4;
    const int bufsz = MT * 4 * plane;
    f32x4 a[MT][4], b0[NT], b1[NT];
#define WINO_MMA(J, B, FIRST)                                                                                   \
    if (!(I2R_DBG(p) & 16))                                                                                     \
    _Pragma("unroll") for (int s = 0; s < 4; ++s) _Pragma("unroll") for (int mt = 0; mt < MT; ++mt)             \
        _Pragma("unroll") for (int nt = 0; nt < NT; ++nt)                                                       \
            acc[J][mt][nt] = mfma16(a[mt][J][s], B[nt][s], ((FIRST) && s == 0) ? (f32x4){0.f, 0.f, 0.f, 0.f} : acc[J][mt][nt]);
#define WINO_PASS(PASS, FIRST)                                                                   \
    {                                                                                            \
        const int pass_ = (PASS);                                                                \
        f32x4* cur = lds + (pass_ & 1) * bufsz;                                                  \
        f32x4* nxt = lds + ((pass_ + 1) & 1) * bufsz;                                            \
        const bool more = pass_ + 1 < npass;                                                     \
        if (more) { stage_load((pass_ + 1) * 16); stage_load_t1((pass_ + 1) * 16); }             \
        load_a(cur, a);                                                                          \
        wp += inc_j; fetch_b(b1);                                                                \
        WINO_MMA(0, b0, FIRST)                                                                   \
        wp += inc_j; fetch_b(b0);                                                                \
        WINO_MMA(1, b1, FIRST)                                                                   \
        if (more) stage_mid((pass_ + 1) * 16);                                                   \
        wp += inc_j; fetch_b(b1);                                                                \
        WINO_MMA(2, b0, FIRST)                                                                   \
        if (more) { wp += inc_wrap; fetch_b(b0); }                                               \
        WINO_MMA(3, b1, FIRST)                                                                   \
        if (more) stage_store(nxt, (pass_ + 1) * 16);                                            \
        if (!(I2R_DBG(p) & 64)) __syncthreads();                                                 \
    }
    stage_load(0);
    stage_load_t1(0);
    if constexpr (FIN) {
        if (fin2) {
            f32x4 vu[NIT];
#pragma unroll
            for (int k = 0; k < NIT; ++k) vu[k] = buf_ld16(rs_t2, goff2[k], 0);
#pragma unroll
            for (int k = 0; k < NIT; ++k) {
                v[k] += vt[k];
                vt[k] = vu[k];
            }
        }
    }
    fetch_b(b0);
    stage_store(lds, 0);
    __syncthreads();
    if (stamp) ts1 = __builtin_amdgcn_s_memtime();
    WINO_PASS(0, true)
    for (int pass = 1; pass < npass; ++pass) WINO_PASS(pass, false)
#undef WINO_PASS
#undef WINO_MMA
    if (stamp) ts2 = __builtin_amdgcn_s_memtime();

    float* const Tl = reinterpret_cast<float*>(lds);
    constexpr int TW = NT * 16;
    constexpr int TPL = MT * 16 * TW;
#pragma unroll
    for (int mt = 0; mt < MT; ++mt)
#pragma unroll
        for (int nt = 0; nt < NT; ++nt) {
            const f32x4 t0 = acc[0][mt][nt] + acc[1][mt][nt] + acc[2][mt][nt];
            const f32x4 t1 = acc[1][mt][nt] - acc[2][mt][nt] - acc[3][mt][nt];
            float* q = Tl + (wi * 2) * TPL + (mt * 16 + 4 * g) * TW + nt * 16 + li;
#pragma unroll
            for (int r = 0; r < 4; ++r) {
                q[r * TW] = t0[r];
                q[TPL + r * TW] = t1[r];
            }
        }
    unsigned obase[MT];
    const int q4 = tid & 3, px = tid >> 2;
    const bool hi = (px & 2) != 0;
    const int n0 = n_base + q4 * 4;
    const bool tail = n_base + NT * 16 > p.cout || n_base + NT * 16 > p.out_cs;
    const unsigned out_bytes = p.out_bytes;
    const __amdgpu_buffer_rsrc_t rs_out = __builtin_amdgcn_make_buffer_rsrc(p.out, 0, out_bytes, 0x00020000);
    const __amdgpu_buffer_rsrc_t rs_r1 = __builtin_amdgcn_make_buffer_rsrc(const_cast<float*>(p.res1), 0, p.res1 ? out_bytes : 0, 0x00020000);
    const __amdgpu_buffer_rsrc_t rs_r2 = __builtin_amdgcn_make_buffer_rsrc(const_cast<float*>(res2), 0, res2 ? out_bytes : 0, 0x00020000);
    const __amdgpu_buffer_rsrc_t rs_rp = __builtin_amdgcn_make_buffer_rsrc(const_cast<float*>(p.res_post), 0, p.res_post ? out_bytes : 0, 0x00020000);
    auto ldb = [](const __amdgpu_buffer_rsrc_t& rs, unsigned off) { return __builtin_bit_cast(f32x4, __builtin_amdgcn_raw_buffer_load_b128(rs, off, 0, 0)); };
    f32x4 r[MT][NT];
#pragma unroll
    for (int mt = 0; mt < MT; ++mt) {
        const int t = px >> 2;
        const int oy = f_oy[mt] + 2 * (t >> fwl) + (hi ? 1 : 0);
        const int ox = f_ox[mt] + 2 * (t & (FW - 1)) + (px & 1);
        const bool ok = f_ok[mt] && oy < p.conv_h && ox < p.conv_w;
        obase[mt] = ok ? (unsigned)(((f_img[mt] * p.out_h + oy) * p.out_w + ox) * p.out_cs + n0) * 4u : kOOB;
#pragma unroll
        for (int k = 0; k < NT; ++k) {
            r[mt][k] = *reinterpret_cast<const f32x4*>(p.bias + n0 + 16 * k);
            if (!(I2R_DBG(p) & 1)) {
                if (p.res1) r[mt][k] += ldb(rs_r1, obase[mt] + 64u * k);
                if (res2) r[mt][k] += ldb(rs_r2, obase[mt] + 64u * k);
            }
        }
    }
    __syncthreads();
    const float* const tq = Tl + ((px & 1) + (hi ? 2 : 0)) * TPL + (px >> 2) * TW + q4 * 4;
    const float sgn = hi ? -1.f : 1.f;
#pragma unroll
    for (int mt = 0; mt < MT; ++mt)
#pragma unroll
        for (int k = 0; k < NT; ++k) {
            const float* q = tq + mt * 16 * TW + 16 * k;
            const f32x4 u0 = *reinterpret_cast<const f32x4*>(q);
            const f32x4 u1 = *reinterpret_cast<const f32x4*>(q + 2 * TPL);
            const f32x4 u2 = *reinterpret_cast<const f32x4*>(q + 4 * TPL);
            f32x4 y = u0 + sgn * (u1 + u2) + r[mt][k];
            if (p.relu) { y[0] = fmaxf(y[0], 0.f); y[1] = fmaxf(y[1], 0.f); y[2] = fmaxf(y[2], 0.f); y[3] = fmaxf(y[3], 0.f); }
            unsigned off = obase[mt] + 64u * k;
            if (p.res_post) y += ldb(rs_rp, off);
            if (tail) {
                const int n = n0 + 16 * k;
                if (!(n + 4 <= p.cout || n + 4 <= p.out_cs)) off = kOOB;
#pragma unroll
                for (int e = 0; e < 4; ++e)
                    if (n + e >= p.cout) y[e] = 0.f;
            }
            if (!(I2R_DBG(p) & 1) || y[0] == 12345.678f) __builtin_amdgcn_raw_buffer_store_b128(__builtin_bit_cast(u32x4, y), rs_out, off, 0, 0);
        }
    if (stamp) {
        asm volatile("s_waitcnt vmcnt(0)" ::: "memory");
        const unsigned long long ts3 = __builtin_amdgcn_s_memtime();
        if (tid == 0) {
            unsigned long long* o = reinterpret_cast<unsigned long long*>(const_cast<float*>(p.res2)) + (size_t)bid * 4;
            o[0] = ts0; o[1] = ts1; o[2] = ts2; o[3] = ts3;
        }
    }
}

template <int MT, int NT>
__global__ __launch_bounds__(256, (MT == 1 ? (NT == 3 ? 4 : 3) : 2)) void conv_wino_f32(const ConvGroupK grp) {
    conv_wino_body<MT, NT, false>(grp);
}

template <int MT, int NT>
__global__ __launch_bounds__(256, (MT == 1 ? (NT == 3 ? 4 : 3) : 2)) void conv_wino_fin_f32(const ConvGroupK grp) {
    conv_wino_body<MT, NT, true>(grp);
}

}

void* i2r_pick_conv_wino(int nt, int mt, int fin) {
    conv_fn fn = nullptr;
    if (mt == 1 && nt == 3) fn = fin ? conv_wino_fin_f32<1, 3> : conv_wino_f32<1, 3>;
    if (mt == 1 && nt == 4) fn = fin ? conv_wino_fin_f32<1, 4> : conv_wino_f32<1, 4>;
    return reinterpret_cast<void*>(fn);
}

size_t i2r_conv_wino_lds(int nt, int mt, int plane) {
    const size_t stage = (size_t)2 * mt * 4 * plane * 16;
    const size_t xchg = (size_t)4 * 2 * mt * 16 * nt * 16 * 4;
    return stage > xchg ? stage : xchg;
}
```

intra-and-inter-human-relation-network-for-mpee_amd/engine.py:

```python
import ctypes as C
import math
import os

import torch

from . import cabi
from .pack import (PRECISIONS, PackedConv, Packer, _m16, _r16, fold_bn, pack_frag, pack_frag32, pack_k4, pack_k8,
                   winograd_weights)


def wino_fragment(conv_h, conv_w):
    best = None
    for fw in (8, 4, 2):
        n = -(-conv_w // (2 * fw)) * -(-conv_h // (32 // fw))
        if best is None or n < best[0]:
            best = (n, 2 * fw, 32 // fw)
    return best[1], best[2]


LP1X1 = True
LP1X1_MAX_PIX = 65536
_HRT_FUSED_ATTN = (78, 156, 312)
_HRT_FUSED_MLP = (78, 156, 312)
_MLP_VARIANT = {78: 1, 156: 2, 312: 2}
PAIR1X1 = True
FUSE_IN = True
PRUNE_FUSE = True
WINOGRAD = True
PROFILER_ATTACHED = bool(os.environ.get("ROCP_TOOL_LIBRARIES") or os.environ.get("ROCPROFILER_LIBRARY_CTOR") or os.environ.get("HSA_TOOLS_LIB")
                         or any(t in os.environ.get("LD_PRELOAD", "") for t in ("rocprof", "roctracer", "rocprofiler")))
DEVICE_SYNC = not PROFILER_ATTACHED


class Act:
    __slots__ = ("t", "n", "h", "w", "c", "cs", "dt")
    TORCH_DT = {0: torch.float32, 1: torch.bfloat16, 2: torch.float16}

    def __init__(self, t, n, h, w, c, cs, dt=0):
        self.t, self.n, self.h, self.w, self.c, self.cs, self.dt = t, n, h, w, c, cs, dt

    def view(self):
        return self.t.view(self.TORCH_DT[self.dt])[:self.n * self.h * self.w * self.cs].view(self.n, self.h, self.w, self.cs)

    @property
    def ptr(self):
        return self.t.data_ptr()


class _RawAct:
    __slots__ = ("ptr", "n", "h", "w", "c", "cs", "dt")

    def __init__(self, ptr, like):
        self.ptr, self.n, self.h, self.w, self.c, self.cs, self.dt = ptr, like.n, like.h, like.w, like.c, like.cs, 0


_MT_EFF = {1: 0.62, 2: 0.9, 3: 1.0, 4: 0.9}


def choose_tile(conv_h, conv_w, wm, stride, max_d, n_img, n_cblk, force_mt=0, want_cost=False):
    best = None
    cands_w = sorted({w for w in (conv_w, 48, 32, 24, 16, 12, 8, 6, 4) if w <= conv_w and w <= 48})
    for mt in ((force_mt,) if force_mt else (1, 2, 3, 4)):
        cap = wm * mt * 16
        for tw in cands_w:
            th = min(conv_h, cap // tw)
            if th < 1:
                continue
            ph, pw = (th - 1) * stride + max_d + 1, (tw - 1) * stride + max_d + 1
            if ph * pw > 1280:
                continue
            tiles = -(-conv_h // th) * -(-conv_w // tw)
            blocks = tiles * n_img * n_cblk
            rounds = -(-blocks // 256)
            halo = ph * pw / float(th * stride * tw * stride)
            cost = rounds * (cap / _MT_EFF[mt]) * (1.0 + 0.08 * (halo - 1.0))
            if best is None or cost < best[0] - 1e-9:
                best = (cost, th, tw, mt)
    assert best is not None, "no tile for %dx%d" % (conv_h, conv_w)
    if want_cost:
        return best
    return best[1], best[2], best[3]


_LPT_CACHE = {}
_LPT_DEV = {}


def lpt_block_table(device, counts, works):
    key = (str(device), tuple(counts), tuple(works))
    t = _LPT_DEV.get(key)
    if t is None:
        ck = (tuple(counts), tuple(works), 256)
        if ck not in _LPT_CACHE:
            _LPT_CACHE[ck] = lpt_block_order(counts, works)
        t = _LPT_DEV[key] = torch.tensor(_LPT_CACHE[ck], dtype=torch.int32, device=device)
    return t


def lpt_block_order(counts, works, n_cu=256):
    import heapq
    items = sorted(((w, g, i) for g, (c, w) in enumerate(zip(counts, works)) for i in range(c)),
                   key=lambda t: (-t[0], t[1], t[2]))
    heap = [(0, b) for b in range(n_cu)]
    bins = [[] for _ in range(n_cu)]
    for w, g, i in items:
        load, b = heapq.heappop(heap)
        bins[b].append((g << 24) | i)
        heapq.heappush(heap, (load + w, b))
    out, r = [], 0
    while len(out) < len(items):
        for b in range(n_cu):
            if r < len(bins[b]):
                out.append(bins[b][r])
        r += 1
    return out


def conv_split(cout_pad):
    nfrag = cout_pad // 16
    nt = next(c for c in (3, 4, 5) if nfrag % c == 0)
    nb = nfrag // nt
    wn = 4 if nb % 4 == 0 else 2 if nb % 2 == 0 else 1
    return nt, wn


class Program:
    def __init__(self, device):
        self.device = device
        self.ops = []
        self.keep = []
        self.pool = {}
        self.pending = []
        self.lane_pool = {}
        self.lane_ctx = 0
        self.groupings = []
        self.enc_stacks = []
        self.split_counters = []
        self.captures = []
        self.query = None
        self.store_dt = 0
        self.in_fork = False
        self.nbytes = 0
        self._snap = None
        self._next_slot = -1
        self._c_ops = None
        self._flags_op = None
        self.uses_lanes = False
        self.device_sync = False
        self._flags = None
        self._events = None
        self._tev = None
        self._capture_ws = None

    def alloc(self, n, h, w, c, dt=0):
        cs = _r16(c)
        numel = (n * h * w * cs + 1) // 2 if dt else n * h * w * cs
        lst = (self.lane_pool.get((self.lane_ctx, numel)) if self.in_fork else None) or self.pool.get(numel)
        if lst:
            t = lst.pop()
        else:
            t = torch.empty(numel, dtype=torch.float32, device=self.device)
            self.nbytes += numel * 4
            self.keep.append(t)
        return Act(t, n, h, w, c, cs, dt)

    def release(self, *acts):
        for a in acts:
            if a is None:
                continue
            if self.in_fork:
                self.lane_pool.setdefault((self.lane_ctx, a.t.numel()), []).append(a.t)
            else:
                self.pool.setdefault(a.t.numel(), []).append(a.t)

    def release_deferred(self, *acts):
        for a in acts:
            if self.in_fork:
                self.pending.append(a.t)
            else:
                self.pool.setdefault(a.t.numel(), []).append(a.t)

    def stem(self, st, n, h, w, in_ptr=0, lane=0, n_src=None, out_dt=0):
        out = self.alloc(n, (h - 1) // 2 + 1, (w - 1) // 2 + 1, st["cout"], out_dt)
        self.keep.append(st)
        ns = n if n_src is None else n_src
        a = cabi.StemArgs(in_ptr, st["w"].data_ptr(), st["bias"].data_ptr(), out.ptr, n, st["cin"], h, w, st["cout"], out.cs, ns, ns, out_dt)
        self.ops.append((cabi.OP_STEM, lane, a))
        return out, a

    def pe_res_stem(self, st, n, h, w, lane=0, n_src=None):
        out = self.alloc(n, (h - 1) // 2 + 1, (w - 1) // 2 + 1, st["cout"])
        self.keep.append(st)
        ns = n if n_src is None else n_src
        a = cabi.PeResArgs(0, st["w_pre"].data_ptr(), st["w7"].data_ptr(), st["bias"].data_ptr(), out.ptr, n, h, w, st["cout"], out.cs, ns, ns)
        self.ops.append((cabi.OP_PE_RES_STEM, lane, a))
        return out, a

    def conv(self, x, pc, relu=False, res1=None, res2=None, res_post=None, in2=None, up=1, out=None, out_step=1,
             out_off=(0, 0), out_hw=None, lane=0, group=None, act=None, out_dt=None, fuse_in=None):
        assert x.cs >= pc.cin_pad and x.c == pc.cin, "conv input channels %d/%d vs weight %d" % (x.c, x.cs, pc.cin)
        assert x.dt in (0, pc.dtype), "16-bit stored input needs the matching 16-bit conv (input %d, conv %d)" % (x.dt, pc.dtype)
        if (LP1X1 and pc.w_lp1 is not None and fuse_in is None and group is None and in2 is None and up == 1 and out_step == 1 and tuple(out_off) == (0, 0)
                and out_hw is None and x.n * x.h * x.w <= LP1X1_MAX_PIX and (out is None or (out.n, out.h, out.w) == (x.n, x.h, x.w))
                and (out is None or out.cs >= pc.cout_pad) and all(r is None or out is None or r.cs == out.cs for r in (res1, res2, res_post))
                and all(r is None or r.cs >= pc.cout_pad for r in (res1, res2, res_post))):
            return self.conv1x1_lp(x, pc, relu=relu, res1=res1, res2=res2, res_post=res_post, out=out, lane=lane, act=act, out_dt=out_dt)
        k = pc.ksize
        if pc.stride == 1:
            conv_h, conv_w = x.h, x.w
        else:
            conv_h, conv_w = (x.h - 1) // 2 + 1, (x.w - 1) // 2 + 1
        if up > 1:
            out_step = up
        if out is None:
            oh, ow = out_hw if out_hw else (conv_h * out_step, conv_w * out_step)
            out = self.alloc(x.n, oh, ow, pc.cout, x.dt if out_dt is None else out_dt)
        assert out.cs >= pc.cout_pad or out.cs >= pc.cout
        assert out.dt in (0, pc.dtype) and all(r is None or r.dt == out.dt for r in (res1, res2, res_post)), "residuals share the output's storage type"
        self._check_like(out, res1, res2, res_post)
        if in2 is not None and (in2.n, in2.h, in2.w, in2.cs) != (x.n, x.h, x.w, x.cs):
            raise ValueError("conv second input is [%d, %d, %d, cs %d], the first [%d, %d, %d, cs %d]" % (in2.n, in2.h, in2.w, in2.cs, x.n, x.h, x.w, x.cs))
        self.keep.append(pc)
        d = cabi.ConvDesc()
        d.in_, d.in2, d.w, d.bias = x.ptr, (in2.ptr if in2 is not None else None), pc.w.data_ptr(), pc.bias.data_ptr()
        d.res1 = res1.ptr if res1 is not None else None
        d.res2 = res2.ptr if res2 is not None else None
        d.res_post = res_post.ptr if res_post is not None else None
        d.out = out.ptr
        d.n_img, d.in_h, d.in_w, d.in_cs, d.cin = x.n, x.h, x.w, x.cs, pc.cin_pad
        d.conv_h, d.conv_w, d.out_h, d.out_w, d.out_cs = conv_h, conv_w, out.h, out.w, out.cs
        d.cout, d.cout_pad, d.stride, d.iy0, d.ix0 = pc.cout, pc.cout_pad, pc.stride, pc.iy0, pc.ix0
        d.ntaps = len(pc.taps)
        for i, (dy, dx) in enumerate(pc.taps):
            d.dy[i], d.dx[i] = dy, dx
        d.out_step, d.out_off_y, d.out_off_x, d.rep = out_step, out_off[0], out_off[1], up
        d.relu = int(relu) if act is None else act
        d.dtype = pc.dtype
        d.in_f16, d.out_f16 = int(x.dt != 0), int(out.dt != 0)
        wino = (WINOGRAD and pc.w_wino is not None and pc.dtype == 0 and in2 is None and up == 1 and out_step == 1 and tuple(out_off) == (0, 0)
                and (out.h, out.w) == (conv_h, conv_w) and d.relu in (0, 1))
        if fuse_in is not None:
            terms, y = fuse_in
            if not (wino and self.fuse_in_ok(x, terms, pc)):
                raise ValueError("fuse_in needs an fp32 Winograd conv over every channel of x and 1 or 2 terms at 1/2 or 1/4 of its map")
            assert all(t.cs == x.cs and t.dt == 0 and t.n == x.n for t in terms) and (y.n, y.h, y.w, y.cs, y.dt) == (x.n, x.h, x.w, x.cs, 0)
            sh = [{2: 1, 4: 2}[x.h // t.h] for t in terms]
            assert all((t.h << k, t.w << k) == (x.h, x.w) for t, k in zip(terms, sh))
            d.t1, d.t1_shift, d.y = terms[0].ptr, sh[0], y.ptr
            if len(terms) > 1:
                d.t2, d.t2_shift = terms[1].ptr, sh[1]
        if wino:
            nfrag = pc.cout_pad // 16
            nt = 3 if nfrag % 3 == 0 else 4
            fw, fh = wino_fragment(conv_h, conv_w)
            d.algo, d.w = 1, pc.w_wino.data_ptr()
            mt = 1
            d.tile_h, d.tile_w, d.mt, d.wn, d.ck = fh, fw, mt, 1, 0
            n_frag = x.n * -(-conv_h // fh) * -(-conv_w // fw)
            geo = ("wino", -(-n_frag // mt) * (nfrag // nt))
            key = ("wino", nt, mt)
        else:
            nt, wn = conv_split(pc.cout_pad)
            n_cblk = (pc.cout_pad // 16) // (nt * wn)
            max_d = max(max(t) for t in pc.taps)
            th, tw, mt = choose_tile(conv_h, conv_w, 4 // wn, pc.stride, max_d, x.n, n_cblk, force_mt=1 if pc.stride == 2 else 0)
            d.tile_h, d.tile_w, d.mt, d.wn, d.ck = th, tw, mt, wn, 0
            geo = (conv_h, conv_w, 4 // wn, pc.stride, max_d, x.n, n_cblk)
            key = nt
        if group is not None:
            group.append((d, geo, key))
        elif wino:
            self.flush_group([(d, geo, key)], lane=lane)
        else:
            self.ops.append((cabi.OP_CONV, lane, d))
        return out

    @staticmethod
    def fuse_in_ok(x, terms, pc):
        return (WINOGRAD and pc.w_wino is not None and pc.dtype == 0 and x.dt == 0 and x.c == pc.cin and x.cs == pc.cin_pad
                and 1 <= len(terms) <= 2 and all((t.h * 2, t.w * 2) == (x.h, x.w) or (t.h * 4, t.w * 4) == (x.h, x.w) for t in terms))

    @staticmethod
    def _group_tiles(group):
        best = None
        s2 = all(geo[3] == 2 for _, geo, _ in group)
        for mt in ((1,) if s2 else (2, 3, 4, 1)):
            try:
                tiles = [choose_tile(*geo, force_mt=mt, want_cost=True) for _, geo, _ in group]
            except AssertionError:
                continue
            blocks = 0
            work = 0.0
            for (d, geo, _), t in zip(group, tiles):
                conv_h, conv_w, wm, stride, max_d, n_img, n_cblk = geo
                nb = -(-conv_h // t[1]) * -(-conv_w // t[2]) * n_img * n_cblk
                blocks += nb
                work += nb * (wm * mt * 16 / _MT_EFF[mt]) * d.cin * d.ntaps
            cost = work * max(1.0, 256.0 / blocks)
            if best is None or cost < best[0]:
                best = (cost, mt, tiles)
        _, mt, tiles = best
        return mt, tiles

    def flush_group(self, group, lane=0):
        if not group:
            return
        nts = {g[2] for g in group}
        wino = group[0][0].algo == 1
        if (len(group) == 1 and not wino) or len(nts) != 1 or len(group) > cabi.MAX_GROUP:
            for m in list(group):
                if m[0].algo == 1:
                    self.flush_group([m], lane=lane)
                else:
                    self.ops.append((cabi.OP_CONV, lane, m[0]))
            del group[:]
            return
        if not wino:
            mt, tiles = self._group_tiles(group)
        order = sorted(range(len(group)), key=lambda i: -(group[i][0].cin * group[i][0].ntaps))
        a = cabi.ConvGroupArgs()
        counts, works = [], []
        for slot, i in enumerate(order):
            d, geo, _ = group[i]
            a.d[slot] = C.pointer(d)
            self.keep.append(d)
            if wino:
                counts.append(geo[1])
            else:
                d.tile_h, d.tile_w, d.mt = tiles[i][1], tiles[i][2], mt
                conv_h, conv_w, wm, stride, max_d, n_img, n_cblk = geo
                counts.append(-(-conv_h // d.tile_h) * -(-conv_w // d.tile_w) * n_img * n_cblk)
            works.append(d.cin * d.ntaps)
        a.n = len(group)
        if not wino and len(set(works)) > 1:
            bm = lpt_block_table(self.device, counts, works)
            self.keep.append(bm)
            a.block_map, a.map_len = bm.data_ptr(), bm.numel()
        self.ops.append((cabi.OP_CONV_GROUP, lane, a))
        del group[:]

    def channel_slice(self, a, c0, c):
        assert c0 % 16 == 0 and c0 + c <= a.cs
        words = c0 // 2 if a.dt else c0
        return Act(a.t[words:], a.n, a.h, a.w, c, a.cs, a.dt)

    def stem_conv2_layer1(self, a, conv2, blocks):
        first = blocks[0]
        assert "c3ds" in first, "layer1.0 carries the downsample"
        cx, cm = conv2.cout, first["c2"].cout
        cat = self.alloc(a.n, (a.h - 1) // 2 + 1, (a.w - 1) // 2 + 1, cx + cm, a.dt)
        x, t2 = self.channel_slice(cat, 0, cx), self.channel_slice(cat, cx, cm)
        self.conv(a, conv2, relu=True, out=x)
        self.release(a)
        t1 = self.conv(x, first["c1"], relu=True)
        self.conv(t1, first["c2"], relu=True, out=t2)
        def pair_ok(pa, pb):
            return (pa.w_frag is not None and pa.cin in (64, 128) and pa.cout % 32 == 0 and pa.cout == pa.cout_pad
                    and (pb is None or (pb.w_frag is not None and pb.cout == 64 and pb.cin == pa.cout)))
        nxt = [b["c1"] for b in blocks[1:]] + [None]
        if PAIR1X1 and a.dt == 0 and pair_ok(first["c3ds"], nxt[0]) and all(pair_ok(b["c3"], nxt[i]) for i, b in enumerate(blocks[1:], 1)):
            self.release(t1)
            y, t1 = self.conv1x1_pair(cat, first["c3ds"], None, blocks[1]["c1"] if len(blocks) > 1 else None)
            self.release(cat)
            for i, blk in enumerate(blocks[1:], 1):
                t2 = self.conv(t1, blk["c2"], relu=True)
                self.release(t1)
                yn, t1 = self.conv1x1_pair(t2, blk["c3"], y, blocks[i + 1]["c1"] if i + 1 < len(blocks) else None)
                self.release(t2, y)
                y = yn
            return y
        y = self.conv(cat, first["c3ds"], relu=True)
        self.release(t1, cat)
        x = y
        for blk in blocks[1:]:
            t1 = self.conv(x, blk["c1"], relu=True)
            t2 = self.conv(t1, blk["c2"], relu=True)
            y = self.conv(t2, blk["c3"], relu=True, res1=x)
            self.release(t1, t2, x)
            x = y
        return x

    def deconv(self, x, pcs, relu=True, res_post=None, lane=0):
        out = self.alloc(x.n, 2 * x.h, 2 * x.w, pcs[(0, 0)].cout, x.dt)
        grp = []
        for (py, px), pc in pcs.items():
            self.conv(x, pc, relu=relu, res_post=res_post, out=out, out_step=2, out_off=(py, px), lane=lane, group=grp)
        self.flush_group(grp, lane=lane)
        return out

    def rows_gather(self, src, crop_map, lane=0):
        out = self.alloc(len(crop_map), src.h, src.w, src.c)
        assert out.cs == src.cs, "rows_gather copies whole rows: source and output need the same row stride (%d vs %d)" % (src.cs, out.cs)
        m = torch.tensor(list(crop_map), dtype=torch.int32).to(self.device)
        self.keep.append(m)
        a = cabi.GatherArgs(src.ptr, out.ptr, m.data_ptr(), len(crop_map), src.h * src.w * src.cs)
        self.ops.append((cabi.OP_ROWS_GATHER, lane, a))
        return out

    def rows_gather_table(self, src, out, table, n_out, src_crop=0, out_crop=0, lane=0):
        per = src.h * src.w * src.cs
        assert src.dt == 0 and out.dt == 0 and (out.h, out.w, out.cs) == (src.h, src.w, src.cs), "rows_gather copies whole fp32 rows of one stride"
        assert table.dtype == torch.int32 and table.numel() >= n_out and 0 <= out_crop and out_crop + n_out <= out.n and 0 <= src_crop < src.n
        self.keep.append(table)
        a = cabi.GatherArgs(src.ptr + 4 * per * src_crop, out.ptr + 4 * per * out_crop, table.data_ptr(), n_out, per)
        self.ops.append((cabi.OP_ROWS_GATHER, lane, a))
        return a

    def view_scramble(self, o, person_map, n_images, max_persons, c, lane=0):
        out = self.alloc(len(person_map), o.h, o.w, c)
        m = torch.tensor(list(person_map), dtype=torch.int32).to(self.device)
        self.keep.append(m)
        a = cabi.ScrambleArgs(o.ptr, out.ptr, m.data_ptr(), len(person_map), n_images, max_persons, c, out.cs, o.h * o.w)
        assert o.cs == out.cs and o.n == n_images * max_persons
        self.ops.append((cabi.OP_VIEW_SCRAMBLE, lane, a))
        return out

    def pe_cat_vec(self, fc, n, h, w, th, tw, out, c0, lane=0, n_src=None):
        rate = int(math.log(w // tw, 2))
        assert (out.n, out.h, out.w) == (n, th, tw) and out.dt == 0 and c0 + fc["vec"] <= out.cs
        self.keep.append(fc)
        ns = n if n_src is None else n_src
        a = cabi.PeCatVecArgs(0, fc["w"].data_ptr(), fc["b"].data_ptr(), out.ptr, n, h, w, th, tw, rate, fc["vec"], out.cs, c0, out.cs, ns, ns)
        self.ops.append((cabi.OP_PE_CAT_VEC, lane, a))
        return a

    def maxpool(self, x, lane=0, out=None):
        assert x.dt == 0, "fp32 kernel: the producer must store fp32 (conv(..., out_dt=0))"
        if out is None:
            out = self.alloc(x.n, (x.h - 1) // 2 + 1, (x.w - 1) // 2 + 1, x.c)
        assert (out.n, out.h, out.w) == (x.n, (x.h - 1) // 2 + 1, (x.w - 1) // 2 + 1) and out.cs >= x.cs and out.dt == 0
        a = cabi.PoolArgs(x.ptr, out.ptr, x.n, x.h, x.w, x.cs, x.cs, out.cs)
        self.ops.append((cabi.OP_MAXPOOL, lane, a))
        return out

    def layernorm(self, x, ln, eps=1e-6, lane=0, out_dt=0):
        assert x.dt == 0, "fp32 kernel: the producer must store fp32 (conv(..., out_dt=0))"
        out = self.alloc(x.n, x.h, x.w, x.c, out_dt)
        self.keep.append(ln)
        a = cabi.LnArgs(x.ptr, ln["w"].data_ptr(), ln["b"].data_ptr(), out.ptr, x.n * x.h * x.w, x.c, x.cs, eps, out_dt)
        self.ops.append((cabi.OP_LAYERNORM, lane, a))
        return out

    def winattn(self, qkv, bias, c, heads, lane=0):
        hs = heads * Packer.HEAD_PAD
        assert qkv.cs == 3 * hs, (qkv.cs, hs)
        out = self.alloc(qkv.n, qkv.h, qkv.w, hs)
        self.keep.append(bias)
        a = cabi.WinAttnArgs(qkv.ptr, bias.data_ptr(), out.ptr, qkv.n, qkv.h, qkv.w, c, hs, heads)
        self.ops.append((cabi.OP_WINATTN, lane, a))
        return out

    def hrt_attn(self, x, ab, eps=1e-6, lane=0, variant=None):
        assert x.dt == 0 and x.c == ab["c"] and x.cs == ab["cs"]
        if not variant or (variant == 1 and ab["c"] not in (78, 156)):
            variant = 2
        out = self.alloc(x.n, x.h, x.w, x.c)
        self.keep.append(ab)
        a = cabi.HrtAttnArgs(x.ptr, out.ptr, ab["ln"]["w"].data_ptr(), ab["ln"]["b"].data_ptr(), ab["wqkv"].data_ptr(), ab["bqkv"].data_ptr(),
                             ab["wo"].data_ptr(), ab["bo"].data_ptr(), x.n, x.h, x.w, x.c, x.cs, ab["heads"], eps, ab["dtype"], variant)
        self.ops.append((cabi.OP_HRT_ATTN, lane, a))
        return out

    def hrt_mlp(self, x, mb, eps=1e-6, lane=0, variant=None):
        assert x.dt == 0 and x.c == mb["c"] and x.cs == mb["cs"]
        if not variant or (variant == 1 and mb["c"] > 156):
            variant = _MLP_VARIANT[mb["c"]]
        out = self.alloc(x.n, x.h, x.w, x.c)
        self.keep.append(mb)
        a = cabi.HrtMlpArgs(x.ptr, out.ptr, mb["ln"]["w"].data_ptr(), mb["ln"]["b"].data_ptr(), mb["w1"].data_ptr(), mb["b1"].data_ptr(),
                            mb["wdw"].data_ptr(), mb["bdw"].data_ptr(), mb["w2"].data_ptr(), mb["b2"].data_ptr(), x.n, x.h, x.w, x.c, x.cs,
                            mb["hidden_pad"], eps, mb["dtype"], variant)
        self.ops.append((cabi.OP_HRT_MLP, lane, a))
        return out

    def dwconv(self, x, dw, stride=1, act=0, lane=0):
        assert x.dt == 0 or stride == 1
        assert x.c == dw["c"] and x.cs == dw["cs"]
        out = self.alloc(x.n, (x.h - 1) // stride + 1, (x.w - 1) // stride + 1, x.c, x.dt)
        self.keep.append(dw)
        a = cabi.DwArgs(x.ptr, dw["w"].data_ptr(), dw["bias"].data_ptr(), out.ptr, x.n, x.h, x.w, x.c, x.cs, stride, act, x.dt)
        self.ops.append((cabi.OP_DWCONV, lane, a))
        return out

    def upsample_add(self, low, res, out, act=0, lane=0):
        lows = list(low) if isinstance(low, (list, tuple)) else [low]
        assert 1 <= len(lows) <= 3
        sc = [out.h // t.h for t in lows]
        assert all(t.h * s == out.h and t.w * s == out.w and t.cs == out.cs == res.cs and t.n == out.n for t, s in zip(lows, sc))
        a = cabi.UpArgs(lows[0].ptr, res.ptr, out.ptr, lows[0].n, lows[0].h, lows[0].w, sc[0], lows[0].c, lows[0].cs, act,
                        lows[1].ptr if len(lows) > 1 else None, lows[2].ptr if len(lows) > 2 else None,
                        sc[1] if len(lows) > 1 else 1, sc[2] if len(lows) > 2 else 1)
        self.ops.append((cabi.OP_UPSAMPLE, lane, a))
        return out

    @staticmethod
    def _check_like(out, *residuals):
        for r in residuals:
            if r is not None and (r.n, r.h, r.w, r.cs) != (out.n, out.h, out.w, out.cs):
                raise ValueError("conv residual is [%d, %d, %d, row %d], the output [%d, %d, %d, row %d]" % (r.n, r.h, r.w, r.cs, out.n, out.h, out.w, out.cs))

    def conv1x1_lp(self, x, pc, relu=False, res1=None, res_post=None, out=None, lane=0, act=None, out_dt=None, res2=None):
        if out is None:
            out = self.alloc(x.n, x.h, x.w, pc.cout, x.dt if out_dt is None else out_dt)
        assert out.cs >= pc.cout_pad and out.dt in (0, pc.dtype) and all(r is None or (r.dt == out.dt and r.cs == out.cs) for r in (res1, res2, res_post))
        self._check_like(out, res1, res2, res_post)
        self.keep.append(pc)
        a = cabi.Conv1x1LpArgs(x.ptr, pc.w_lp1.data_ptr(), pc.bias.data_ptr(), res1.ptr if res1 is not None else None,
                               res_post.ptr if res_post is not None else None, out.ptr, x.n * x.h * x.w, pc.cin_pad, pc.cout_pad, x.cs, out.cs,
                               (int(relu) if act is None else act), pc.dtype, int(x.dt != 0), int(out.dt != 0), 0,
                               res2.ptr if res2 is not None else None)
        self.ops.append((cabi.OP_CONV1X1_LP, lane, a))
        return out

    def conv1x1_pair(self, x, pa, res, pb, lane=0):
        assert x.dt == 0 and pa.w_frag is not None and pa.ksize == 1 and pa.cin == x.cs and (pb is None or (pb.w_frag is not None and pb.cin == pa.cout))
        y = self.alloc(x.n, x.h, x.w, pa.cout)
        z = self.alloc(x.n, x.h, x.w, pb.cout) if pb is not None else None
        assert res is None or (res.cs == y.cs and res.dt == 0 and res.n * res.h * res.w == y.n * y.h * y.w)
        self.keep.extend([pa, pb])
        a = cabi.Conv1x1PairArgs(x.ptr, pa.w_frag.data_ptr(), pa.bias.data_ptr(), res.ptr if res is not None else None, y.ptr,
                                 pb.w_frag.data_ptr() if pb is not None else None, pb.bias.data_ptr() if pb is not None else None,
                                 z.ptr if z is not None else None, x.n * x.h * x.w, pa.cin, pa.cout, pb.cout if pb is not None else 0,
                                 x.cs, y.cs, z.cs if z is not None else 0, 1, 1, 0)
        self.ops.append((cabi.OP_CONV1X1_PAIR, lane, a))
        return y, z

    def fuse_up_add(self, base, terms, out, relu=True, lane=0):
        assert 1 <= len(terms) <= 2 and all(t.cs == base.cs == out.cs and t.dt == base.dt == out.dt and t.n == base.n for t in terms)
        sc = [base.h // t.h for t in terms]
        assert all(t.h * s == base.h and t.w * s == base.w for t, s in zip(terms, sc))
        a = cabi.FuseUpArgs(base.ptr, terms[0].ptr, terms[1].ptr if len(terms) > 1 else None, out.ptr, base.n, base.h, base.w, base.cs,
                            sc[0], sc[1] if len(terms) > 1 else 1, int(relu), base.dt)
        self.ops.append((cabi.OP_FUSE_UP, lane, a))
        return out

    def head(self, x, hd, out_ptr=0, lane=0):
        assert x.dt == 0, "fp32 kernel: the producer must store fp32 (conv(..., out_dt=0))"
        self.keep.append(hd)
        tmp = None
        if hd.get("conv3") is not None:
            x = tmp = self.conv(x, hd["conv3"], out_dt=0, lane=lane)
        a = cabi.HeadArgs(x.ptr, hd["w"].data_ptr(), hd["bias"].data_ptr(), out_ptr, x.n, x.h, x.w, hd["cin"], x.cs, hd["cout"])
        self.ops.append((cabi.OP_HEAD, lane, a))
        if tmp is not None:
            self.release(tmp)
        return a

    def encoder(self, x, layers, grp_off_host, pos=None, pos_period=0, lane=0, regroupable=False, pre_norm=False, pos_table=None, capture=None):
        assert x.dt == 0, "the encoder kernels read fp32 token rows"
        if layers and layers[0].get("mh"):
            return self.encoder_mh(x, layers, grp_off_host, pos=pos, pos_period=pos_period, lane=lane, regroupable=regroupable, pre_norm=pre_norm,
                                   pos_table=pos_table, capture=capture)
        assert not pre_norm, "the fused layer kernels are post-norm"
        cap = self._capture_begin(capture, x)
        pos_act = self._pos_rows(x, pos, pos_period, pos_table) if cap is not None else None
        n_tok = x.n * x.h * x.w
        cs = x.cs
        n_pad = (n_tok + 63) // 64 * 64 + 64
        fuse_kv = all(not L.get("dtype", 0) for L in layers) and len(layers) > 1
        nbuf = 2 if fuse_kv else 1
# ... 1688 lines not shown
```

Baseline: 8720 images/sec.

## Run several Winograd fragments sequentially per workgroup for small-cin convs

Winograd conv workgroups now loop over up to 8 consecutive fragments instead of one. The count is chosen per group member from cin so that each workgroup covers enough channel passes, and it is reduced again while the total grid would fall below 512 workgroups. This amortises per-workgroup setup (descriptor reads, resource construction, index math) and launch overhead for shallow-cin convs. Per-fragment parameters are re-read from the kernarg segment to keep register pressure down. The cost is fewer workgroups, so occupancy can drop, and an extra barrier between fragments.

```diff
diff --git a/include/i2r_hip.h b/include/i2r_hip.h
--- a/include/i2r_hip.h
+++ b/include/i2r_hip.h
@@ -50,6 +50,7 @@
     const float* t1;
     const float* t2;
     float* y;
+    int32_t seq;
 } i2r_conv_desc;
 
 I2R_API int i2r_conv(const i2r_conv_desc* d, void* stream);
@@ -78,6 +79,8 @@
              int32_t w_, int32_t cin, int32_t in_cs, int32_t cout, void* stream);
 
 I2R_API int i2r_conv_kernel_name(const i2r_conv_desc* const* descs, int32_t n, char* buf, int32_t buflen);
+
+I2R_API int i2r_conv_grid(const i2r_conv_desc* const* descs, int32_t n, int32_t with_map, int32_t* grid, int32_t* seq);
 
 I2R_API int i2r_flip_merge(const float* y, const float* y_flipped, const int32_t* joint_map, float* out, int32_t n, int32_t joints,
                    int32_t h, int32_t w, void* stream);
diff --git a/intra-and-inter-human-relation-network-for-mpee_amd/cabi.py b/intra-and-inter-human-relation-network-for-mpee_amd/cabi.py
--- a/intra-and-inter-human-relation-network-for-mpee_amd/cabi.py
+++ b/intra-and-inter-human-relation-network-for-mpee_amd/cabi.py
@@ -43,6 +43,7 @@
         ("tile_h", _i32), ("tile_w", _i32), ("ck", _i32), ("wn", _i32), ("mt", _i32), ("dtype", _i32),
         ("in_f16", _i32), ("out_f16", _i32), ("algo", _i32),
         ("t1_shift", _i32), ("t2_shift", _i32), ("t1", _fp), ("t2", _fp), ("y", _fp),
+        ("seq", _i32),
     ]
 
 
@@ -217,7 +218,7 @@
     _fields_ = [("kind", _i32), ("lane", _i32), ("args", C.c_void_p)]
 
 
-EXPORTS = ("i2r_conv", "i2r_conv_grouped", "i2r_conv_kernel_name", "i2r_stem_conv", "i2r_pe_res_stem", "i2r_maxpool3x3s2", "i2r_head", "i2r_layernorm", "i2r_window_attn", "i2r_hrt_attn_block", "i2r_hrt_mlp_block", "i2r_dwconv3x3",
+EXPORTS = ("i2r_conv", "i2r_conv_grouped", "i2r_conv_kernel_name", "i2r_conv_grid", "i2r_stem_conv", "i2r_pe_res_stem", "i2r_maxpool3x3s2", "i2r_head", "i2r_layernorm", "i2r_window_attn", "i2r_hrt_attn_block", "i2r_hrt_mlp_block", "i2r_dwconv3x3",
            "i2r_upsample_bilinear_add", "i2r_upsample_bilinear_add_multi", "i2r_fuse_up_add", "i2r_conv1x1_pair", "i2r_conv1x1_lp", "i2r_flip_merge", "i2r_decode", "i2r_pose_nms", "i2r_group_nearest", "i2r_oks_match", "i2r_oks_accumulate", "i2r_joint_targets", "i2r_val_metrics", "i2r_crop_affine", "i2r_box_mask", "i2r_crop_affine_cv2", "i2r_box_mask_cv2", "i2r_person_inputs_cv2", "i2r_encoder_kv", "i2r_encoder_layer", "i2r_mh_attention", "i2r_attn_weights", "i2r_attn_query_maps", "i2r_pe_cat_vec", "i2r_rows_gather", "i2r_view_scramble",
            "i2r_run_program", "i2r_run_program_timed", "i2r_abi_version", "i2r_last_error", "i2r_device_check")
 
@@ -237,6 +238,7 @@
     L.i2r_conv.argtypes = [C.POINTER(ConvDesc), C.c_void_p]
     L.i2r_conv_grouped.argtypes = [C.POINTER(C.POINTER(ConvDesc)), _i32, _fp, _i32, C.c_void_p]
     L.i2r_conv_kernel_name.argtypes = [C.POINTER(C.POINTER(ConvDesc)), _i32, C.c_char_p, _i32]
+    L.i2r_conv_grid.argtypes = [C.POINTER(C.POINTER(ConvDesc)), _i32, _i32, C.POINTER(_i32), C.POINTER(_i32)]
     L.i2r_stem_conv.argtypes = [_fp, _fp, _fp, _fp, _i32, _i32, _i32, _i32, _i32, _i32, _i32, _i32, _i32, C.c_void_p]
     L.i2r_pe_res_stem.argtypes = [_fp, _fp, _fp, _fp, _fp, _i32, _i32, _i32, _i32, _i32, _i32, _i32, C.c_void_p]
     L.i2r_flip_merge.argtypes = [_fp, _fp, _fp, _fp, _i32, _i32, _i32, _i32, C.c_void_p]
diff --git a/intra-and-inter-human-relation-network-for-mpee_amd/csrc/i2r_conv.h b/intra-and-inter-human-relation-network-for-mpee_amd/csrc/i2r_conv.h
--- a/intra-and-inter-human-relation-network-for-mpee_amd/csrc/i2r_conv.h
+++ b/intra-and-inter-human-relation-network-for-mpee_amd/csrc/i2r_conv.h
@@ -34,6 +34,7 @@
     unsigned in_bytes, w_bytes, out_bytes;
     int wn_log, npass;
     int algo, w_fwlog, w_pitch, w_half, w_nfrag, w_rcp;
+    int w_seq;
     int w_band;
     unsigned w_m_cblk, w_m_img, w_m_tx;
     const float* f_t1;
diff --git a/intra-and-inter-human-relation-network-for-mpee_amd/csrc/i2r_conv.hip b/intra-and-inter-human-relation-network-for-mpee_amd/csrc/i2r_conv.hip
--- a/intra-and-inter-human-relation-network-for-mpee_amd/csrc/i2r_conv.hip
+++ b/intra-and-inter-human-relation-network-for-mpee_amd/csrc/i2r_conv.hip
@@ -270,12 +270,17 @@
     k.out_step = d->out_step; k.out_off_y = d->out_off_y; k.out_off_x = d->out_off_x; k.rep = d->rep; k.relu = d->relu;
     k.dtype = d->dtype;
     k.in16 = d->in_f16; k.out16 = d->out_f16;
-    k.algo = d->algo; k.w_fwlog = k.w_pitch = k.w_half = k.w_nfrag = k.w_rcp = k.w_band = 0;
+    k.algo = d->algo; k.w_fwlog = k.w_pitch = k.w_half = k.w_nfrag = k.w_rcp = k.w_band = 0; k.w_seq = 1;
     k.w_m_cblk = k.w_m_img = k.w_m_tx = 0; k.in_bytes = k.w_bytes = k.out_bytes = 0;
     k.m_cblk = k.m_tx = k.m_ty = k.m_pw = k.m_tw = 0; k.wn_log = 0; k.npass = 0;
     k.dbg = 0;
     k.f_t1 = d->t1; k.f_t2 = d->t2; k.f_y = d->y; k.f_sh1 = d->t1_shift; k.f_sh2 = d->t2 ? d->t2_shift : 0; k.f_bytes1 = k.f_bytes2 = 0;
 }
+
+constexpr int kWinoMaxSeq = 8;
+constexpr int kWinoRunPasses = 6;
+constexpr int kWinoMinWg = 512;
+static long long wino_runs(const ConvK& k, int mt) { return (((long long)k.w_nfrag + mt - 1) / mt + k.w_seq - 1) / k.w_seq; }
 
 static int prepare_wino(const i2r_conv_desc* d, int force_mt, ConvK& k, int* nt_out, int* mt_out, int* cap_out, int* pf_out, size_t* lds_out,
                         long long* nblk_out) {
@@ -306,6 +311,7 @@
     I2R_CHECK_ARG(nt != 0, "i2r_conv: algo 1 needs cout_pad=%d to be a multiple of 48 or 64", d->cout_pad);
     const int mt = force_mt ? force_mt : (d->mt ? d->mt : 1);
     I2R_CHECK_ARG(mt == 1, "i2r_conv: algo 1 takes mt 1 (got %d)", mt);
+    I2R_CHECK_ARG(d->seq >= 0 && d->seq <= kWinoMaxSeq, "i2r_conv: algo 1 runs 1..%d fragments per workgroup (seq=%d; 0 = choose)", kWinoMaxSeq, d->seq);
     int fw = 0;
     if (d->tile_w) {
         I2R_CHECK_ARG(d->tile_w == 16 || d->tile_w == 8 || d->tile_w == 4, "i2r_conv: algo 1 fragment width %d (16, 8, 4)", d->tile_w);
@@ -339,6 +345,7 @@
     const long long nf = (long long)d->n_img * k.tiles_y * k.tiles_x;
     I2R_CHECK_ARG(nf > 0 && nf * k.n_cblk < (1ll << 20) && k.tiles_y * k.tiles_x < 2048 && k.n_cblk < 2048, "i2r_conv: algo 1 grid (%lld fragments)", nf);
     k.w_nfrag = (int)nf;
+    k.w_seq = d->seq ? d->seq : 1;
 #ifdef I2R_TUNING
     {
         static const int dbg = getenv("I2R_CONV_DBG") ? atoi(getenv("I2R_CONV_DBG")) : 0;
@@ -347,8 +354,27 @@
 #endif
     *nt_out = nt; *mt_out = mt; *cap_out = 0; *pf_out = 100;
     *lds_out = i2r_conv_wino_lds(nt, mt, k.plane);
-    *nblk_out = (nf + mt - 1) / mt * k.n_cblk;
+    *nblk_out = wino_runs(k, mt) * k.n_cblk;
     return I2R_OK;
+}
+
+static void wino_choose_seq(ConvK* g, const i2r_conv_desc* const* descs, int n, int mt) {
+    auto total = [&]() { long long t = 0; for (int i = 0; i < n; ++i) t += wino_runs(g[i], mt) * g[i].n_cblk; return t; };
+    long long at_one = 0;
+    for (int i = 0; i < n; ++i) at_one += ((long long)g[i].w_nfrag + mt - 1) / mt * g[i].n_cblk;
+    const long long floor_wg = std::min<long long>(at_one, kWinoMinWg);
+    for (int i = 0; i < n; ++i)
+        if (descs[i]->seq == 0) g[i].w_seq = std::max(1, std::min(kWinoMaxSeq, kWinoRunPasses / (g[i].cin >> 4)));
+    while (total() < floor_wg) {
+        int pick = -1;
+        for (int i = 0; i < n; ++i) {
+            if (descs[i]->seq != 0 || g[i].w_seq == 1) continue;
+            const int len = g[i].w_seq * (g[i].cin >> 4);
+            if (pick < 0 || len > g[pick].w_seq * (g[pick].cin >> 4) || (len == g[pick].w_seq * (g[pick].cin >> 4) && g[i].cin > g[pick].cin)) pick = i;
+        }
+        if (pick < 0) break;
+        --g[pick].w_seq;
+    }
 }
 
 static int prepare(const i2r_conv_desc* d, int force_mt, int force_cap, int force_pf, ConvK& k, int* nt_out, int* mt_out, int* cap_out,
@@ -537,13 +563,22 @@
         I2R_CHECK_ARG(nt == nt0 && mt == mt0, "i2r_conv_grouped: descriptor %d has fragment blocking (%d,%d) != (%d,%d)", i, mt, nt, mt0, nt0);
         I2R_CHECK_ARG(descs[i]->dtype == descs[0]->dtype, "i2r_conv_grouped: members mix compute dtypes");
         if (lds > lds_max) lds_max = lds;
-        if (descs[i]->algo == 1 && !table) {
-            const long long groups = nblk / grp.g[i].n_cblk;
-            grp.g[i].w_band = (int)((groups + 7) / 8);
-            nblk = (long long)grp.g[i].w_band * 8 * grp.g[i].n_cblk;
-        }
+        if (descs[i]->algo == 1) continue;
         total += nblk;
         grp.blk_end[i] = (int)total;
+    }
+    if (descs[0]->algo == 1) {
+        wino_choose_seq(grp.g, descs, n, mt0);
+        for (int i = 0; i < n; ++i) {
+            const long long runs = wino_runs(grp.g[i], mt0);
+            long long nblk = runs * grp.g[i].n_cblk;
+            if (!table) {
+                grp.g[i].w_band = (int)((runs + 7) / 8);
+                nblk = (long long)grp.g[i].w_band * 8 * grp.g[i].n_cblk;
+            }
+            total += nblk;
+            grp.blk_end[i] = (int)total;
+        }
     }
     for (int i = n; i < kMaxGroups; ++i) { grp.g[i] = grp.g[0]; grp.blk_end[i] = (int)total; }
     grp.n = n;
@@ -582,6 +617,20 @@
 
 extern "C" int i2r_conv(const i2r_conv_desc* d, void* stream) { return i2r_conv_grouped(&d, 1, nullptr, 0, stream); }
 
+extern "C" int i2r_conv_grid(const i2r_conv_desc* const* descs, int32_t n, int32_t with_map, int32_t* grid, int32_t* seq) {
+    ConvGroupK grp;
+    int nt0, mt0, cap0, pf0;
+    size_t lds_max;
+    long long total;
+    int rc = resolve(descs, n, grp, &nt0, &mt0, &cap0, &pf0, &lds_max, &total, with_map != 0);
+    if (rc) return rc;
+    I2R_CHECK_ARG(grid != nullptr, "i2r_conv_grid: grid");
+    *grid = (int32_t)total;
+    if (seq)
+        for (int i = 0; i < n; ++i) seq[i] = descs[0]->algo == 1 ? grp.g[i].w_seq : 1;
+    return I2R_OK;
+}
+
 extern "C" int i2r_conv_kernel_name(const i2r_conv_desc* const* descs, int32_t n, char* buf, int32_t buflen) {
     ConvGroupK grp;
     int nt0, mt0, cap0, pf0;
diff --git a/intra-and-inter-human-relation-network-for-mpee_amd/csrc/i2r_conv_wino.hip b/intra-and-inter-human-relation-network-for-mpee_amd/csrc/i2r_conv_wino.hip
--- a/intra-and-inter-human-relation-network-for-mpee_amd/csrc/i2r_conv_wino.hip
+++ b/intra-and-inter-human-relation-network-for-mpee_amd/csrc/i2r_conv_wino.hip
@@ -4,8 +4,10 @@
 
 constexpr int kWinoPatchMax = 108;
 
+typedef const ConvK __attribute__((address_space(4)))* ConvKArg;
+
 template <int MT, int NT, bool FIN>
-__device__ __forceinline__ void conv_wino_body(const ConvGroupK& grp) {
+__device__ __forceinline__ void conv_wino_body(const ConvGroupK& grp, ConvKArg args) {
     extern __shared__ __attribute__((aligned(16))) f32x4 lds[];
     const int tid = threadIdx.x, lane = tid & 63;
     const int wi = __builtin_amdgcn_readfirstlane(tid >> 6);
@@ -27,7 +29,6 @@
     const bool stamp = (I2R_DBG(p) & 8) != 0;
     unsigned long long ts0 = 0, ts1 = 0, ts2 = 0;
     if (stamp) ts0 = __builtin_amdgcn_s_memtime();
-    const float* const res2 = stamp ? nullptr : p.res2;
 
     int wg, cb;
     if (grp.blk_map) {
@@ -37,68 +38,83 @@
         const int q = bid >> 3, qq = div_m(q, p.n_cblk, p.w_m_cblk);
         cb = q - qq * p.n_cblk;
         wg = (bid & 7) * p.w_band + qq;
-        if (wg * MT >= p.w_nfrag) return;
-    }
+    }
+    const int run0 = wg * p.w_seq;
+    const int nrun = min(p.w_seq, (p.w_nfrag + MT - 1) / MT - run0);
+    if (nrun <= 0) return;
     const int fwl = p.w_fwlog, FW = 1 << fwl;
-    const int PC = p.pw, PP = p.ph * p.pw;
-    const int per_img = p.tiles_y * p.tiles_x;
     const int pitch = p.w_pitch, half = p.w_half, plane = p.plane;
     const int n_base = cb * NT * 16;
-    int f_img[MT], f_oy[MT], f_ox[MT];
-    bool f_ok[MT];
-#pragma unroll
-    for (int mt = 0; mt < MT; ++mt) {
-        int fid = wg * MT + mt;
-        f_ok[mt] = fid < p.w_nfrag;
-        if (!f_ok[mt]) fid = 0;
-        f_img[mt] = div_m(fid, per_img, p.w_m_img);
-        const int rem = fid - f_img[mt] * per_img;
-        const int fy = div_m(rem, p.tiles_x, p.w_m_tx);
-        f_oy[mt] = fy * (32 >> fwl);
-        f_ox[mt] = (rem - fy * p.tiles_x) * (2 * FW);
-    }
 
     constexpr int NIT = (MT * kWinoPatchMax * 4 + 255) / 256;
     const __amdgpu_buffer_rsrc_t rs_in = __builtin_amdgcn_make_buffer_rsrc(const_cast<float*>(p.in), 0, p.in_bytes, 0x00020000);
     const __amdgpu_buffer_rsrc_t rs_w = __builtin_amdgcn_make_buffer_rsrc(const_cast<float*>(p.w), 0, p.w_bytes, 0x00020000);
     unsigned goff[NIT];
     int lslot[NIT];
+    constexpr int kOwn = 1 << 30;
     const bool fin = FIN && p.f_t1 != nullptr, fin2 = fin && p.f_t2 != nullptr;
     const __amdgpu_buffer_rsrc_t rs_t1 = make_rsrc(fin ? p.f_t1 : nullptr, p.f_bytes1), rs_t2 = make_rsrc(fin2 ? p.f_t2 : nullptr, p.f_bytes2),
                                  rs_y = make_rsrc(fin ? p.f_y : nullptr, p.in_bytes);
     unsigned goff1[FIN ? NIT : 1], goff2[FIN ? NIT : 1];
-    bool own[FIN ? NIT : 1];
-#pragma unroll
-    for (int k = 0; k < NIT; ++k) {
-        const int it = tid + k * 256;
-        const int cg = it & 3, pix = it >> 2;
-        int f = 0, pp = pix;
+    const int cg = tid & 3;
+    auto patch_pixel = [&](const auto& pq, int t, int k, int& f, int& row, int& col) {
+        const int PC = pq.pw, PP = pq.ph * pq.pw;
+        const int pix = (t + k * 256) >> 2;
+        int pp = pix;
+        f = 0;
 #pragma unroll
         for (int m = 1; m <= MT; ++m)
             if (pix >= m * PP) { f = m; pp = pix - m * PP; }
-        const int row = (pp * p.w_rcp) >> 16, col = pp - row * PC;
-        goff[k] = kOOB;
-        lslot[k] = -1;
-        if constexpr (FIN) { goff1[k] = goff2[k] = kOOB; own[k] = false; }
-        if (f < MT) {
+        row = (pp * pq.w_rcp) >> 16;
+        col = pp - row * PC;
+    };
+#pragma unroll
+    for (int k = 0; k < NIT; ++k) {
+        int f, row, col;
+        patch_pixel(p, tid, k, f, row, col);
+        lslot[k] = f < MT ? (f * 4 + cg) * plane + row * pitch + (col & 1) * half + (col >> 1) : -1;
+        if constexpr (FIN) {
+            if (f < MT && row >= 1 && row < p.ph - 1 && col >= 1 && col < p.pw - 1) lslot[k] |= kOwn;
+        }
+    }
+    auto lane_now = []() {
+        int l;
+        asm volatile("v_mbcnt_lo_u32_b32 %0, -1, 0\n\tv_mbcnt_hi_u32_b32 %0, -1, %0" : "=v"(l));
+        return l;
+    };
+    int f_img[MT], f_oy[MT], f_ox[MT];
+    bool f_ok[MT];
+    auto set_fragment = [&](int fg, int t, const auto& ps) {
+#pragma unroll
+        for (int mt = 0; mt < MT; ++mt) {
+            int fid = fg * MT + mt;
+            f_ok[mt] = fid < ps.w_nfrag;
+            if (!f_ok[mt]) fid = 0;
+            f_img[mt] = div_m(fid, (ps.tiles_y * ps.tiles_x), ps.w_m_img);
+            const int rem = fid - f_img[mt] * (ps.tiles_y * ps.tiles_x);
+            const int fy = div_m(rem, ps.tiles_x, ps.w_m_tx);
+            f_oy[mt] = fy * (32 >> fwl);
+            f_ox[mt] = (rem - fy * ps.tiles_x) * (2 * FW);
+        }
+#pragma unroll
+        for (int k = 0; k < NIT; ++k) {
+            int f, row, col;
+            patch_pixel(ps, t, k, f, row, col);
             int img = f_img[0], oy = f_oy[0], ox = f_ox[0];
-            bool ok = f_ok[0];
+            bool ok = f_ok[0] && f < MT;
 #pragma unroll
             for (int m = 1; m < MT; ++m)
                 if (f == m) { img = f_img[m]; oy = f_oy[m]; ox = f_ox[m]; ok = f_ok[m]; }
             const int iy = oy - 1 + row, ix = ox - 1 + col;
-            lslot[k] = (f * 4 + cg) * plane + row * pitch + (col & 1) * half + (col >> 1);
-            if (ok && iy >= 0 && iy < p.in_h && ix >= 0 && ix < p.in_w) {
-                goff[k] = (unsigned)(((img * p.in_h + iy) * p.in_w + ix) * p.in_cs + cg * 4) * 4u;
-                if constexpr (FIN) {
-                    const int s1 = p.f_sh1, s2 = p.f_sh2;
-                    goff1[k] = (unsigned)(((img * (p.in_h >> s1) + (iy >> s1)) * (p.in_w >> s1) + (ix >> s1)) * p.in_cs + cg * 4) * 4u;
-                    goff2[k] = (unsigned)(((img * (p.in_h >> s2) + (iy >> s2)) * (p.in_w >> s2) + (ix >> s2)) * p.in_cs + cg * 4) * 4u;
-                    own[k] = row >= 1 && row < p.ph - 1 && col >= 1 && col < PC - 1;
-                }
-            }
-        }
-    }
+            const bool in_img = ok && (unsigned)iy < (unsigned)ps.in_h && (unsigned)ix < (unsigned)ps.in_w;
+            goff[k] = in_img ? (unsigned)(((img * ps.in_h + iy) * ps.in_w + ix) * ps.in_cs + (t & 3) * 4) * 4u : kOOB;
+            if constexpr (FIN) {
+                const int s1 = ps.f_sh1, s2 = ps.f_sh2;
+                goff1[k] = in_img ? (unsigned)(((img * (ps.in_h >> s1) + (iy >> s1)) * (ps.in_w >> s1) + (ix >> s1)) * ps.in_cs + (t & 3) * 4) * 4u : kOOB;
+                goff2[k] = in_img ? (unsigned)(((img * (ps.in_h >> s2) + (iy >> s2)) * (ps.in_w >> s2) + (ix >> s2)) * ps.in_cs + (t & 3) * 4) * 4u : kOOB;
+            }
+        }
+    };
     f32x4 v[NIT];
     auto stage_load = [&](int c0) {
 #pragma unroll
@@ -133,13 +149,13 @@
                 for (int k = 0; k < NIT; ++k) {
                     v[k] += vt[k];
                     v[k][0] = fmaxf(v[k][0], 0.f); v[k][1] = fmaxf(v[k][1], 0.f); v[k][2] = fmaxf(v[k][2], 0.f); v[k][3] = fmaxf(v[k][3], 0.f);
-                    if (cb == 0) buf_st16(rs_y, own[k] ? goff[k] : kOOB, c0 * 4, v[k]);
+                    if (cb == 0) buf_st16(rs_y, (unsigned)lslot[k] >= (unsigned)kOwn ? goff[k] : kOOB, c0 * 4, v[k]);
                 }
             }
         }
 #pragma unroll
         for (int k = 0; k < NIT; ++k)
-            if (lslot[k] >= 0) buf[lslot[k]] = v[k];
+            if (lslot[k] >= 0) buf[FIN ? lslot[k] & (kOwn - 1) : lslot[k]] = v[k];
     };
 
     const int ra = wi == 0 ? 0 : (wi == 2 ? 2 : 1);
@@ -147,11 +163,12 @@
     const float sg = wi == 1 ? 1.f : -1.f;
     const int ty = li >> fwl, tx = li & (FW - 1);
     const int abase = g * plane + 2 * ty * pitch + tx;
+    int abase_f;
     const int oa = ra * pitch, ob = rb * pitch;
     auto load_a = [&](const f32x4* buf, f32x4 (&a)[MT][4]) {
 #pragma unroll
         for (int mt = 0; mt < MT; ++mt) {
-            const f32x4* q = buf + mt * 4 * plane + abase;
+            const f32x4* q = buf + mt * 4 * plane + abase_f;
             f32x4 R[4];
 #pragma unroll
             for (int c = 0; c < 4; ++c) {
@@ -168,7 +185,8 @@
 
     const int cin4 = p.cin >> 2;
     const unsigned wlane = (unsigned)(n_base + li + g * p.cout_pad) * 16u;
-    int wp = wi * 4 * cin4 * p.cout_pad * 16;
+    const int wp0 = wi * 4 * cin4 * p.cout_pad * 16;
+    int wp;
     const int inc_j = cin4 * p.cout_pad * 16;
     const int inc_wrap = (4 - 3 * cin4) * p.cout_pad * 16;
     auto fetch_b = [&](f32x4 (&b)[NT]) {
@@ -206,6 +224,23 @@
         if (more) stage_store(nxt, (pass_ + 1) * 16);                                            \
         if (!(I2R_DBG(p) & 64)) __syncthreads();                                                 \
     }
+    float* const Tl = reinterpret_cast<float*>(lds);
+    constexpr int TW = NT * 16;
+    constexpr int TPL = MT * 16 * TW;
+    const bool tail = n_base + NT * 16 > p.cout || n_base + NT * 16 > p.out_cs;
+
+    for (int fs = 0; fs < nrun; ++fs) {
+    {
+        const int tid_s = wi * 64 + lane_now();
+        ConvKArg ps_ = args + gi;
+        asm volatile("" : "+s"(ps_));
+        set_fragment(run0 + fs, tid_s, *ps_);
+        abase_f = abase;
+        asm volatile("" : "+v"(abase_f));
+#pragma unroll
+        for (int k = 0; k < NIT; ++k) asm volatile("" : "+v"(lslot[k]));
+    }
+    wp = wp0;
     stage_load(0);
     stage_load_t1(0);
     if constexpr (FIN) {
@@ -221,25 +256,29 @@
         }
     }
     fetch_b(b0);
+    if (fs) __syncthreads();
     stage_store(lds, 0);
     __syncthreads();
     if (stamp) ts1 = __builtin_amdgcn_s_memtime();
     WINO_PASS(0, true)
     for (int pass = 1; pass < npass; ++pass) WINO_PASS(pass, false)
-#undef WINO_PASS
-#undef WINO_MMA
     if (stamp) ts2 = __builtin_amdgcn_s_memtime();
 
-    float* const Tl = reinterpret_cast<float*>(lds);
-    constexpr int TW = NT * 16;
-    constexpr int TPL = MT * 16 * TW;
+    const int tid_f = wi * 64 + lane_now();
+    ConvKArg pe_ = args + gi;
+    asm volatile("" : "+s"(pe_));
+    const auto& pe = *pe_;
+    const float* const res2e = stamp ? nullptr : pe.res2;
+    const unsigned out_bytes = pe.out_bytes;
+    const __amdgpu_buffer_rsrc_t rs_out = make_rsrc(pe.out, out_bytes), rs_r1 = make_rsrc(pe.res1, out_bytes), rs_r2 = make_rsrc(res2e, out_bytes),
+                                 rs_rp = make_rsrc(pe.res_post, out_bytes);
 #pragma unroll
     for (int mt = 0; mt < MT; ++mt)
 #pragma unroll
         for (int nt = 0; nt < NT; ++nt) {
             const f32x4 t0 = acc[0][mt][nt] + acc[1][mt][nt] + acc[2][mt][nt];
             const f32x4 t1 = acc[1][mt][nt] - acc[2][mt][nt] - acc[3][mt][nt];
-            float* q = Tl + (wi * 2) * TPL + (mt * 16 + 4 * g) * TW + nt * 16 + li;
+            float* q = Tl + (wi * 2) * TPL + (mt * 16 + ((tid_f & 63) >> 4) * 4) * TW + nt * 16 + (tid_f & 15);
 #pragma unroll
             for (int r = 0; r < 4; ++r) {
                 q[r * TW] = t0[r];
@@ -247,36 +286,29 @@
             }
         }
     unsigned obase[MT];
-    const int q4 = tid & 3, px = tid >> 2;
+    const int q4 = tid_f & 3, px = tid_f >> 2;
     const bool hi = (px & 2) != 0;
     const int n0 = n_base + q4 * 4;
-    const bool tail = n_base + NT * 16 > p.cout || n_base + NT * 16 > p.out_cs;
-    const unsigned out_bytes = p.out_bytes;
-    const __amdgpu_buffer_rsrc_t rs_out = __builtin_amdgcn_make_buffer_rsrc(p.out, 0, out_bytes, 0x00020000);
-    const __amdgpu_buffer_rsrc_t rs_r1 = __builtin_amdgcn_make_buffer_rsrc(const_cast<float*>(p.res1), 0, p.res1 ? out_bytes : 0, 0x00020000);
-    const __amdgpu_buffer_rsrc_t rs_r2 = __builtin_amdgcn_make_buffer_rsrc(const_cast<float*>(res2), 0, res2 ? out_bytes : 0, 0x00020000);
-    const __amdgpu_buffer_rsrc_t rs_rp = __builtin_amdgcn_make_buffer_rsrc(const_cast<float*>(p.res_post), 0, p.res_post ? out_bytes : 0, 0x00020000);
-    auto ldb = [](const __amdgpu_buffer_rsrc_t& rs, unsigned off) { return __builtin_bit_cast(f32x4, __builtin_amdgcn_raw_buffer_load_b128(rs, off, 0, 0)); };
     f32x4 r[MT][NT];
 #pragma unroll
     for (int mt = 0; mt < MT; ++mt) {
         const int t = px >> 2;
         const int oy = f_oy[mt] + 2 * (t >> fwl) + (hi ? 1 : 0);
         const int ox = f_ox[mt] + 2 * (t & (FW - 1)) + (px & 1);
-        const bool ok = f_ok[mt] && oy < p.conv_h && ox < p.conv_w;
-        obase[mt] = ok ? (unsigned)(((f_img[mt] * p.out_h + oy) * p.out_w + ox) * p.out_cs + n0) * 4u : kOOB;
+        const bool ok = f_ok[mt] && oy < pe.conv_h && ox < pe.conv_w;
+        obase[mt] = ok ? (unsigned)(((f_img[mt] * pe.out_h + oy) * pe.out_w + ox) * pe.out_cs + n0) * 4u : kOOB;
 #pragma unroll
         for (int k = 0; k < NT; ++k) {
-            r[mt][k] = *reinterpret_cast<const f32x4*>(p.bias + n0 + 16 * k);
+            r[mt][k] = *reinterpret_cast<const f32x4*>(pe.bias + n0 + 16 * k);
             if (!(I2R_DBG(p) & 1)) {
-                if (p.res1) r[mt][k] += ldb(rs_r1, obase[mt] + 64u * k);
-                if (res2) r[mt][k] += ldb(rs_r2, obase[mt] + 64u * k);
-            }
-        }
-    }
-    __syncthreads();
+                if (pe.res1) r[mt][k] += buf_ld16(rs_r1, obase[mt] + 64u * k, 0);
+                if (res2e) r[mt][k] += buf_ld16(rs_r2, obase[mt] + 64u * k, 0);
+            }
+        }
+    }
     const float* const tq = Tl + ((px & 1) + (hi ? 2 : 0)) * TPL + (px >> 2) * TW + q4 * 4;
     const float sgn = hi ? -1.f : 1.f;
+    __syncthreads();
 #pragma unroll
     for (int mt = 0; mt < MT; ++mt)
 #pragma unroll
@@ -286,18 +318,21 @@
             const f32x4 u1 = *reinterpret_cast<const f32x4*>(q + 2 * TPL);
             const f32x4 u2 = *reinterpret_cast<const f32x4*>(q + 4 * TPL);
             f32x4 y = u0 + sgn * (u1 + u2) + r[mt][k];
-            if (p.relu) { y[0] = fmaxf(y[0], 0.f); y[1] = fmaxf(y[1], 0.f); y[2] = fmaxf(y[2], 0.f); y[3] = fmaxf(y[3], 0.f); }
+            if (pe.relu) { y[0] = fmaxf(y[0], 0.f); y[1] = fmaxf(y[1], 0.f); y[2] = fmaxf(y[2], 0.f); y[3] = fmaxf(y[3], 0.f); }
             unsigned off = obase[mt] + 64u * k;
-            if (p.res_post) y += ldb(rs_rp, off);
+            if (pe.res_post) y += buf_ld16(rs_rp, off, 0);
             if (tail) {
                 const int n = n0 + 16 * k;
-                if (!(n + 4 <= p.cout || n + 4 <= p.out_cs)) off = kOOB;
+                if (!(n + 4 <= pe.cout || n + 4 <= pe.out_cs)) off = kOOB;
 #pragma unroll
                 for (int e = 0; e < 4; ++e)
-                    if (n + e >= p.cout) y[e] = 0.f;
+                    if (n + e >= pe.cout) y[e] = 0.f;
             }
             if (!(I2R_DBG(p) & 1) || y[0] == 12345.678f) __builtin_amdgcn_raw_buffer_store_b128(__builtin_bit_cast(u32x4, y), rs_out, off, 0, 0);
         }
+    }
+#undef WINO_PASS
+#undef WINO_MMA
     if (stamp) {
         asm volatile("s_waitcnt vmcnt(0)" ::: "memory");
         const unsigned long long ts3 = __builtin_amdgcn_s_memtime();
@@ -308,14 +343,19 @@
     }
 }
 
+__device__ __forceinline__ ConvKArg wino_args() {
+    static_assert(offsetof(ConvGroupK, g) == 0, "the members lead the kernel argument");
+    return (ConvKArg)__builtin_amdgcn_kernarg_segment_ptr();
+}
+
 template <int MT, int NT>
 __global__ __launch_bounds__(256, (MT == 1 ? (NT == 3 ? 4 : 3) : 2)) void conv_wino_f32(const ConvGroupK grp) {
-    conv_wino_body<MT, NT, false>(grp);
+    conv_wino_body<MT, NT, false>(grp, wino_args());
 }
 
 template <int MT, int NT>
 __global__ __launch_bounds__(256, (MT == 1 ? (NT == 3 ? 4 : 3) : 2)) void conv_wino_fin_f32(const ConvGroupK grp) {
-    conv_wino_body<MT, NT, true>(grp);
+    conv_wino_body<MT, NT, true>(grp, wino_args());
 }
 
 }
diff --git a/intra-and-inter-human-relation-network-for-mpee_amd/engine.py b/intra-and-inter-human-relation-network-for-mpee_amd/engine.py
--- a/intra-and-inter-human-relation-network-for-mpee_amd/engine.py
+++ b/intra-and-inter-human-relation-network-for-mpee_amd/engine.py
@@ -27,6 +27,7 @@
 FUSE_IN = True
 PRUNE_FUSE = True
 WINOGRAD = True
+WINO_SEQ = True
 PROFILER_ATTACHED = bool(os.environ.get("ROCP_TOOL_LIBRARIES") or os.environ.get("ROCPROFILER_LIBRARY_CTOR") or os.environ.get("HSA_TOOLS_LIB")
                          or any(t in os.environ.get("LD_PRELOAD", "") for t in ("rocprof", "roctracer", "rocprofiler")))
 DEVICE_SYNC = not PROFILER_ATTACHED
@@ -256,6 +257,7 @@
             d.algo, d.w = 1, pc.w_wino.data_ptr()
             mt = 1
             d.tile_h, d.tile_w, d.mt, d.wn, d.ck = fh, fw, mt, 1, 0
+            d.seq = 0 if WINO_SEQ else 1
             n_frag = x.n * -(-conv_h // fh) * -(-conv_w // fw)
             geo = ("wino", -(-n_frag // mt) * (nfrag // nt))
             key = ("wino", nt, mt)
```

After: 8827 images/sec, median of 6. +1.2%, better.
